# asharakeh/bayes-od-rc

Measured on AMD Instinct MI355X. Metric: images/sec at N=10 MC samples, 512x512; per-anchor covariance latency, higher is better.
Workload: dtype bf16; 1 GPU; ResNet-50 RetinaNet + covar head, N=10 MC-dropout, 512x512, full BayesOD pipeline (forward+posterior+soft-NMS+cluster-fuse); global_batch=512, mc_samples=10, anchors=49104, parallelism=one GPU (no exchange; N > 1: image-sharded, one RCCL gather/step), visible_gpus=1, gpu_max_hw_queues=4

## Files before the change

### bayes-od-rc_amd/_lib.py

```python
import ctypes as C
import os

import numpy as np


_HERE = os.path.dirname(os.path.abspath(__file__))
LIB_PATH = os.path.join(_HERE, "lib", "libbayesod_hip.so")
if os.environ.get("BOD_LIB_OVERRIDE"):
    LIB_PATH = os.path.abspath(os.environ["BOD_LIB_OVERRIDE"])

BOD_OK, BOD_ERR_INVALID_ARG, BOD_ERR_HIP, BOD_ERR_OOM, BOD_ERR_NOT_READY, BOD_ERR_NO_DEVICE = range(6)


class BodConfig(C.Structure):
    _fields_ = [
        ("device", C.c_int32), ("image_h", C.c_int32), ("image_w", C.c_int32), ("batch", C.c_int32),
        ("mc_samples", C.c_int32), ("num_classes", C.c_int32), ("anchors_per_location", C.c_int32),
        ("min_level", C.c_int32), ("max_level", C.c_int32), ("dropout_rate", C.c_float),
        ("use_full_covar", C.c_int32), ("dirichlet_non_informative", C.c_int32),
        ("gaussian_isotropic", C.c_int32), ("isotropic_variance", C.c_float),
        ("ranking_method", C.c_int32), ("nms_max_output_size", C.c_int32),
        ("nms_iou_threshold", C.c_float), ("nms_soft_sigma", C.c_float), ("nms_variant", C.c_int32),
        ("num_categorical_draws", C.c_int32), ("has_covar_head", C.c_int32),
        ("kitti_scale_h", C.c_float), ("kitti_scale_w", C.c_float), ("precision", C.c_int32),
        ("mc_sample_base", C.c_int32),
        ("mc_ensemble_size", C.c_int32),
        ("training", C.c_int32),
        ("backbone_depth", C.c_int32),
        ("pipeline_overlap", C.c_int32),
        ("reserved", C.c_int32 * 2),
    ]


class BodSizes(C.Structure):
    _fields_ = [
        ("num_pixels", C.c_int32), ("num_anchors", C.c_int32), ("level_h", C.c_int32 * 8),
        ("level_w", C.c_int32 * 8), ("num_levels", C.c_int32), ("max_detections", C.c_int32),
        ("device_bytes", C.c_int64),
    ]


_F = C.POINTER(C.c_float)
_I = C.POINTER(C.c_int32)
_H = C.c_void_p

SIGNATURES = {
    "bod_version": (C.c_char_p, []),
    "bod_last_error": (C.c_char_p, [_H]),
    "bod_create": (C.c_int, [C.POINTER(BodConfig), C.POINTER(_H)]),
    "bod_destroy": (C.c_int, [_H]),
    "bod_query_sizes": (C.c_int, [_H, C.POINTER(BodSizes)]),
    "bod_update_config": (C.c_int, [_H, C.POINTER(BodConfig)]),
    "bod_load_weight": (C.c_int, [_H, C.c_char_p, C.c_int32, C.POINTER(C.c_int64), C.c_int32, _F]),
    "bod_finalize_weights": (C.c_int, [_H]),
    "bod_set_anchors": (C.c_int, [_H, _F, C.c_int32]),
    "bod_forward": (C.c_int, [_H, C.c_void_p, C.c_int32, C.c_uint64, C.c_uint32]),
    "bod_get_raw": (C.c_int, [_H, _F, _F, _F]),
    "bod_set_raw": (C.c_int, [_H, _F, _F, _F]),
    "bod_get_pyramid": (C.c_int, [_H, C.c_int32, _F]),
    "bod_posterior": (C.c_int, [_H, C.c_uint64, C.c_uint32]),
    "bod_validation_post": (C.c_int, [_H]),
    "bod_get_num_kept": (C.c_int, [_H, _I]),
    "bod_get_posterior": (C.c_int, [_H, C.c_int32, _F, _F, _F, _F, _F, _I]),
    "bod_set_posterior": (C.c_int, [_H, C.c_int32, C.c_int32, _F, _F, _F, _F]),
    "bod_nms": (C.c_int, [_H]),
    "bod_get_nms": (C.c_int, [_H, C.c_int32, _I, _I]),
    "bod_set_nms": (C.c_int, [_H, C.c_int32, _I, C.c_int32]),
    "bod_get_iou_matrix": (C.c_int, [_H, C.c_int32, _F]),
    "bod_cluster_fuse": (C.c_int, [_H]),
    "bod_set_affinity": (C.c_int, [_H, C.c_int32, _F, C.c_int32, C.c_int32]),
    "bod_get_detections": (C.c_int, [_H, C.c_int32, _I, _F, _F, _F, _F]),
    "bod_get_detections_batch": (C.c_int, [_H, _I, _F, _F, _F, _F]),
    "bod_device_detections": (C.c_int, [_H, C.c_int32, C.POINTER(C.c_void_p)]),
    "bod_device_raw": (C.c_int, [_H, C.POINTER(C.c_void_p), C.c_int32]),
    "bod_infer": (C.c_int, [_H, C.c_void_p, C.c_int32, C.c_uint64, C.c_uint32]),
    "bod_infer_async": (C.c_int, [_H, C.c_void_p, C.c_int32, C.c_uint64, C.c_uint32, _I]),
    "bod_collect": (C.c_int, [_H, C.c_int32, _I, _F, _F, _F, _F]),
    "bod_upload_images": (C.c_int, [_H, _F]),
    "bod_upload_frames_u8": (C.c_int, [_H, C.POINTER(C.c_uint8), C.c_int32, C.c_int32, _F, C.c_int32]),
    "bod_upload_frames_u8_async": (C.c_int, [_H, C.POINTER(C.c_uint8), C.c_int32, C.c_int32, _F, C.c_int32, C.c_int32]),
    "bod_device_images_buffer": (C.c_void_p, [_H, C.c_int32]),
    "bod_device_images": (C.c_void_p, [_H]),
    "bod_synchronize": (C.c_int, [_H]),
    "bod_stage_conv_wgrad": (C.c_int, [C.c_int32, _F, C.c_int32, C.c_int32, C.c_int32, C.c_int32, _F, C.c_int32, C.c_int32,
                                       C.c_int32, C.c_int32, C.c_int32, C.c_int32, _F, _F]),
    "bod_stage_conv": (C.c_int, [C.c_int32, _F, C.c_int32, C.c_int32, C.c_int32, C.c_int32, _F, _F,
                                 C.c_int32, C.c_int32, C.c_int32, C.c_int32, C.c_int32, C.c_int32, _F,
                                 C.c_float, C.c_uint64, C.c_int32, C.c_uint32, C.c_int32, C.c_int32, _F]),
    "bod_loss_forward": (C.c_int, [C.c_int32, C.c_int32, C.c_int32, C.c_int32, _F, _F, _F, _F, _F, _F,
                                   C.POINTER(C.c_uint8), C.POINTER(C.c_uint8), C.c_int32, C.c_int32, C.c_float,
                                   C.POINTER(C.c_double)]),
    "bod_train_step": (C.c_int, [_H, C.c_void_p, C.c_int32, _F, _F, C.POINTER(C.c_uint8), C.POINTER(C.c_uint8), C.c_uint64, C.c_uint32,
                                 C.c_int32, C.c_float, C.c_float, C.c_float, C.c_float, C.c_float, C.c_int32, C.POINTER(C.c_double)]),
    "bod_train_gradients": (C.c_int, [_H, C.POINTER(C.c_void_p), C.POINTER(C.c_int64)]),
    "bod_train_apply": (C.c_int, [_H, C.c_float, C.POINTER(C.c_double)]),
    "bod_train_get": (C.c_int, [_H, C.c_char_p, C.c_int32, C.c_int32, _F, C.c_int64]),
    "bod_train_set": (C.c_int, [_H, C.c_char_p, C.c_int32, C.c_int32, _F, C.c_int64]),
    "bod_train_step_count": (C.c_int, [_H, C.POINTER(C.c_int64), C.c_int64]),
    "bod_loss_backward": (C.c_int, [C.c_int32, C.c_int32, C.c_int32, C.c_int32, _F, _F, _F, _F, _F, _F,
                                    C.POINTER(C.c_uint8), C.POINTER(C.c_uint8), C.c_int32, C.c_int32, C.c_float,
                                    C.c_float, C.c_float, C.POINTER(C.c_double), _F, _F, _F]),
    "bod_bench_head_conv": (C.c_int, [_H, C.c_int32, C.c_int32, C.c_int32, C.POINTER(C.c_double), C.POINTER(C.c_double)]),
    "bod_profile_begin": (C.c_int, [_H]),
    "bod_profile_select": (C.c_int, [_H, C.c_int32]),
    "bod_plan_info": (C.c_int, [_H, C.POINTER(C.c_int32)]),
    "bod_record_width": (C.c_int32, [_H]),
    "bod_gather_detections": (C.c_int, [_H, C.c_int32, C.c_void_p, C.c_int32, C.c_int32, C.c_int32, C.c_void_p, C.POINTER(C.c_void_p)]),
    "bod_profile_end": (C.c_int, [_H, C.POINTER(C.c_double), C.POINTER(C.c_int64),
                                  C.POINTER(C.c_double), C.POINTER(C.c_double), C.POINTER(C.c_int64)]),
}

_lib = None


def load():
    global _lib
    if _lib is not None:
        return _lib
    if not os.path.exists(LIB_PATH):
        raise RuntimeError(
            "libbayesod_hip.so not found at %s -- build it with `python -c 'import __graft_entry__ as g; "
            "g.build()'` (there is no CPU fallback)" % LIB_PATH)
    lib = C.CDLL(LIB_PATH)
    for name, (res, args) in SIGNATURES.items():
        fn = getattr(lib, name)
        fn.restype = res
        fn.argtypes = args
    _lib = lib
    return lib


def fptr(a):
    return None if a is None else a.ctypes.data_as(_F)


def iptr(a):
    return None if a is None else a.ctypes.data_as(_I)


def check(lib, handle, status):
    if status == BOD_OK:
        return
    msg = lib.bod_last_error(handle)
    msg = msg.decode() if msg else "status %d" % status
    if status in (BOD_ERR_INVALID_ARG, BOD_ERR_NOT_READY):
        raise ValueError(msg)
    if status == BOD_ERR_OOM:
        raise MemoryError(msg)
    raise RuntimeError(msg)


def as_f32(a):
    return np.ascontiguousarray(a, dtype=np.float32)
```

### bayes-od-rc_amd/csrc/engine.hip

```cpp
#include "../../include/bayesod.h"
#include "kernels.h"

#include <algorithm>
#include <atomic>
#include <cmath>
#include <condition_variable>
#include <deque>
#include <functional>
#include <mutex>
#include <thread>
#include <tuple>
#include <cstdarg>
#include <cstdio>
#include <cstring>
#include <map>
#include <memory>
#include <string>
#include <vector>
#include <dlfcn.h>

namespace {

constexpr float BN_EPS = 1e-3f;

thread_local std::string g_create_error;

struct HostTensor { std::vector<int64_t> shape; std::vector<float> data; };

struct Plane {
    char* d = nullptr;
    int64_t base = 0;
    int64_t bstride = 0;
    int h = 0, w = 0, C = 0, pitch = 0;
};

struct PackedConv { char* w = nullptr; float* bias = nullptr; int cout = 0, cout_pad = 0, taps = 0, kw = 0, cin = 0; };

struct Op {
    enum Kind { STEM, POOL, CONV, KEEP } kind;
    ConvArgs conv;
    bool is_head3x3 = false;
    double flops = 0;
    std::string name;
    std::string wname[3], bnname[3];
    bool same_geom = false;
    int flavour = 0;
    int head[3] = {-1, -1, -1};
    bool hx_pyramid = false;
};
enum { FLAVOUR_BOTH = 0, FLAVOUR_RAW = 1, FLAVOUR_AGG = 2 };

uint16_t f2bf(float f) {
    uint32_t u; std::memcpy(&u, &f, 4);
    u += 0x7FFFu + ((u >> 16) & 1u);
    return (uint16_t)(u >> 16);
}
float bf2f(uint16_t v) { uint32_t u = (uint32_t)v << 16; float f; std::memcpy(&f, &u, 4); return f; }

uint16_t f2h(float f) {
    uint32_t u; std::memcpy(&u, &f, 4);
    const uint32_t sign = (u >> 16) & 0x8000u;
    u &= 0x7FFFFFFFu;
    if (u >= 0x47800000u) return (uint16_t)(sign | (u > 0x7F800000u ? 0x7E00u : 0x7C00u));
    if (u < 0x38800000u) {
        float a; std::memcpy(&a, &u, 4);
        return (uint16_t)(sign | (uint32_t)std::nearbyint(a * 16777216.0f));
    }
    u += 0xFFFu + ((u >> 13) & 1u);
    return (uint16_t)(sign | ((u - 0x38000000u) >> 13));
}
float h2f(uint16_t h) {
    const uint32_t sign = (uint32_t)(h & 0x8000u) << 16, e = (h >> 10) & 31u, m = h & 0x3FFu;
    float f;
    if (e == 0) { f = (float)m * (1.0f / 16777216.0f); uint32_t u; std::memcpy(&u, &f, 4); u |= sign; std::memcpy(&f, &u, 4); return f; }
    const uint32_t u = sign | ((e == 31 ? 255u : e + 112u) << 23) | (m << 13);
    std::memcpy(&f, &u, 4);
    return f;
}
uint32_t f2e2m3(float x) {
    const uint32_t sign = std::signbit(x) ? 32u : 0u;
    const float a = std::fabs(x);
    uint32_t code;
    if (a < 1.0f) code = (uint32_t)std::nearbyint(a * 8.0f);
    else if (a < 2.0f) code = 8u + (uint32_t)std::nearbyint((a - 1.0f) * 8.0f);
    else if (a < 4.0f) code = 16u + (uint32_t)std::nearbyint((a - 2.0f) * 4.0f);
    else code = 24u + (uint32_t)std::nearbyint((std::min(a, 7.5f) - 4.0f) * 2.0f);
    return sign | std::min(code, 31u);
}
float e2m3_to_f(uint32_t c) {
    const uint32_t e = (c >> 3) & 3u, m = c & 7u;
    const float r = e == 0 ? m / 8.0f : std::ldexp(1.0f + m / 8.0f, (int)e - 1);
    return (c & 32u) ? -r : r;
}
void pack_hx_row(const float* v, int C, uint8_t* dst, bool weights) {
    std::memset(dst, 0, (size_t)C * 4);
    for (int q = 0; q < C / 64; ++q) {
        uint8_t* H = dst + (size_t)q * 256;
        uint8_t* X = H + 128;
        for (int c = 0; c < 64; ++c) { const uint16_t hb = f2h(v[q * 64 + c]); std::memcpy(H + 2 * c, &hb, 2); }
        for (int m = 0; m < 2; ++m)
            for (int b = 0; b < 2; ++b) {
                float hi[16], lo[16], mx = 6.103515625e-05f;
                for (int k = 0; k < 16; ++k) {
                    const float x = v[q * 64 + 32 * m + 8 * (k >> 2) + 4 * b + (k & 3)];
                    hi[k] = h2f(f2h(x)); lo[k] = (x - hi[k]) * 2048.0f;
                    mx = std::max(mx, std::fabs(x));
                }
                const float mxs = mx * 1.0666667f;
                uint32_t ub; std::memcpy(&ub, &mxs, 4);
                const uint32_t eb = (ub >> 23) - 2u;
                const float inv = std::ldexp(1.0f, 127 - (int)eb);
                uint8_t slot[32] = {0};
                for (int k = 0; k < 16; ++k) {
                    const uint32_t h6 = f2e2m3(hi[k] * inv), l6 = f2e2m3(lo[k] * inv);
                    const uint32_t e0 = weights ? l6 : h6, e1 = weights ? h6 : l6;
                    const int bit0 = 12 * k;
                    for (int t = 0; t < 6; ++t) {
                        if ((e0 >> t) & 1u) slot[(bit0 + t) >> 3] |= (uint8_t)(1u << ((bit0 + t) & 7));
                        if ((e1 >> t) & 1u) slot[(bit0 + 6 + t) >> 3] |= (uint8_t)(1u << ((bit0 + 6 + t) & 7));
                    }
                }
                slot[28] = (uint8_t)(weights ? eb - 11u : eb);
                std::memcpy(X + 64 * m + 16 * b, slot, 16);
                std::memcpy(X + 64 * m + 32 + 16 * b, slot + 16, 16);
            }
    }
}
void unpack_hx_row(const uint8_t* src, int C, float* v) {
    for (int q = 0; q < C / 64; ++q) {
        const uint8_t* H = src + (size_t)q * 256;
        const uint8_t* X = H + 128;
        for (int m = 0; m < 2; ++m)
            for (int b = 0; b < 2; ++b) {
                uint8_t slot[32];
                std::memcpy(slot, X + 64 * m + 16 * b, 16);
                std::memcpy(slot + 16, X + 64 * m + 32 + 16 * b, 16);
                const float sc = std::ldexp(1.0f, (int)slot[28] - 127);
                for (int k = 0; k < 16; ++k) {
                    const int c = 32 * m + 8 * (k >> 2) + 4 * b + (k & 3);
                    uint16_t hb; std::memcpy(&hb, H + 2 * c, 2);
                    uint32_t l6 = 0;
                    for (int t = 0; t < 6; ++t) l6 |= (uint32_t)((slot[(12 * k + 6 + t) >> 3] >> ((12 * k + 6 + t) & 7)) & 1u) << t;
                    v[q * 64 + c] = h2f(hb) + e2m3_to_f(l6) * sc * (1.0f / 2048.0f);
                }
            }
    }
}

uint32_t f2e2m1(float x) {
    const uint32_t s = std::signbit(x) ? 8u : 0u;
    float a = std::fabs(x);
    if (!(a == a)) return s;
    if (a >= 6.0f) return s | 7u;
    static const float grid[8] = {0.f, 0.5f, 1.f, 1.5f, 2.f, 3.f, 4.f, 6.f};
    uint32_t best = 0;
    for (uint32_t c = 0; c < 7; ++c) {
        const float mid = 0.5f * (grid[c] + grid[c + 1]);
        if (a > mid || (a == mid && (c & 1u))) best = c + 1;
    }
    return s | best;
}
float e2m1_to_f(uint32_t c) {
    static const float grid[8] = {0.f, 0.5f, 1.f, 1.5f, 2.f, 3.f, 4.f, 6.f};
    return (c & 8u) ? -grid[c & 7u] : grid[c & 7u];
}
void pack_h4_row(const float* v, int C, uint8_t* dst, bool weights) {
    std::memset(dst, 0, (size_t)C * 4);
    for (int q = 0; q < C / 64; ++q) {
        uint8_t* H = dst + (size_t)(3 * (q >> 1) + (q & 1)) * 128;
        for (int c = 0; c < 64; ++c) { const uint16_t hb = f2h(v[q * 64 + c]); std::memcpy(H + 2 * c, &hb, 2); }
    }
    for (int x = 0; x < C / 128; ++x)
        for (int ks = 0; ks < 4; ++ks)
            for (int b = 0; b < 2; ++b) {
                float hi[16], lo[16], mx = 6.103515625e-05f;
                for (int k = 0; k < 16; ++k) {
                    const float xv = v[128 * x + 32 * ks + 8 * (k >> 2) + 4 * b + (k & 3)];
                    hi[k] = h2f(f2h(xv)); lo[k] = (xv - hi[k]) * 2048.0f;
                    mx = std::max(mx, std::fabs(hi[k]));
                }
                const float mxs = mx * 1.3333334f;
                uint32_t ub; std::memcpy(&ub, &mxs, 4);
                const uint32_t eb = (ub >> 23) - 2u;
                const float inv = std::ldexp(1.0f, 127 - (int)eb);
                uint8_t* piece = dst + (size_t)(3 * x + 2) * 128 + (2 * ks + b) * 16;
                for (int k = 0; k < 16; ++k) {
                    const uint32_t h4 = f2e2m1(hi[k] * inv), l4 = f2e2m1(lo[k] * inv);
                    piece[k] = (uint8_t)(weights ? (l4 | (h4 << 4)) : (h4 | (l4 << 4)));
                }
                dst[6 * 128 + 8 * x + 4 * b + ks] = (uint8_t)(weights ? eb - 11u : eb);
            }
}
void unpack_h4_row(const uint8_t* src, int C, float* v) {
    for (int x = 0; x < C / 128; ++x)
        for (int ks = 0; ks < 4; ++ks)
            for (int b = 0; b < 2; ++b) {
                const uint8_t* piece = src + (size_t)(3 * x + 2) * 128 + (2 * ks + b) * 16;
                const float sc = std::ldexp(1.0f, (int)src[6 * 128 + 8 * x + 4 * b + ks] - 127);
                for (int k = 0; k < 16; ++k) {
                    const int c = 128 * x + 32 * ks + 8 * (k >> 2) + 4 * b + (k & 3);
                    const int q = c >> 6;
                    uint16_t hb; std::memcpy(&hb, src + (size_t)(3 * (q >> 1) + (q & 1)) * 128 + 2 * (c & 63), 2);
                    v[c] = h2f(hb) + e2m1_to_f((uint32_t)piece[k] >> 4) * sc * (1.0f / 2048.0f);
                }
            }
}

}

struct bod_context {
    bod_config cfg{};
    std::string err;
    hipStream_t stream = nullptr;
    std::vector<void*> allocs;
    std::map<const void*, size_t> alloc_bytes;
    int64_t device_bytes = 0;
    struct TrainState* train = nullptr;

    int sh = 0, sw = 0, ph = 0, pw = 0;
    int ch[6] = {0}, cw[6] = {0};
    int nlev = 0; int lh[8] = {0}, lw[8] = {0};
    int64_t lvl_off[8] = {0};
    int64_t lvl_p0[8] = {0};
    int64_t Ppad = 0; int P = 0, A = 0;

    std::map<std::string, HostTensor> host_w;
    std::map<std::string, PackedConv> packed;
    float* stem_w = nullptr; float* stem_b = nullptr;
    bool weights_ready = false, anchors_ready = false, forward_done = false, posterior_done = false,
         nms_done = false, cluster_done = false;

    float* d_images = nullptr;
    float* splitk_partial = nullptr; size_t splitk_elems = 0;
    uint8_t* d_frames_u8 = nullptr; size_t frames_u8_cap = 0;
    float* d_images_b[2] = {nullptr, nullptr}; uint8_t* d_u8_b[2] = {nullptr, nullptr}; size_t u8_cap_b[2] = {0, 0};
    hipStream_t copy = nullptr;
    hipEvent_t ev_img_ready[2] = {nullptr, nullptr}, ev_img_free[2] = {nullptr, nullptr};
    bool img_ready_pending[2] = {false, false}, img_free_pending[2] = {false, false};
    int cur_img_buf = -1;
    char* stem_out = nullptr;
    int es = 2;
    bool split = false;
    char* pyr_hx = nullptr;
    int pyr_fmt = 1;
    int plan_mx = 0;
    int mx = 0;
    Plane pyramid;
    char* head_act[3][2] = {{nullptr}};
    char* head_act_t[3][4] = {{nullptr}};
    float* raw[3] = {nullptr};
    float* agg[3] = {nullptr};
    bool agg_plan = false;
    bool plan_fused_out = false, plan_xreuse = false, plan_xreuse0 = false;
    bool raw_valid = false, agg_valid = false;
    bool plan_sparse = false;
    SparseTailArgs sparse{};
    bool agg_sparse = false;
    bool keep_ready = false;
    uint64_t keep_seed = 0; uint32_t keep_first = 0;
    uint64_t last_seed = 0; uint32_t last_first_image = 0;
    std::map<std::string, RowEnt*> tables;
    struct XrTable { RowEnt* rows = nullptr; int2* ext = nullptr; int m = 0; };
    std::map<std::string, XrTable> xr_tables;
    std::vector<Op> ops;
    const float* cur_images = nullptr;

    float* d_anchors = nullptr;
    PostBuffers pb{};
    float* nms_scores = nullptr; int32_t* nms_begin = nullptr;
    int32_t* nms_sel_s[2] = {nullptr, nullptr}; int32_t* nms_nsel_s[2] = {nullptr, nullptr};
    float* out_scores_s[2] = {nullptr, nullptr}; float* out_means_s[2] = {nullptr, nullptr};
    float* out_covs_s[2] = {nullptr, nullptr}; float* out_counts_s[2] = {nullptr, nullptr};
    int32_t* nms_sel = nullptr; int32_t* nms_nsel = nullptr;
    float* out_scores = nullptr; float* out_means = nullptr; float* out_covs = nullptr; float* out_counts = nullptr;
    int slot = 0;
    hipStream_t side = nullptr;
    int overlap_mode = 0;
    int ov_front_slots = 0, ov_slots = 0;
    hipStream_t full = nullptr, front = nullptr, back = nullptr;
    hipEvent_t ev_front_done[2] = {nullptr, nullptr}, ev_l0_done[2] = {nullptr, nullptr}, ev_join = nullptr;
    bool l0_pending[2] = {false, false};
    bool ov_dirty = false;
    char* pyr_d[2] = {nullptr, nullptr};
    int fwd_parity = 0, pyr_last = 0;
    int first_head_op = 0;
    bool in_overlap_call = false;
    int n_cu = 256;
    hipEvent_t ev_posterior = nullptr; hipEvent_t ev_done[2] = {nullptr, nullptr};
    int dev_op_lo = 0, dev_op_hi = 1 << 30;
    hipStream_t done_stream[2] = {nullptr, nullptr};
    bool side_pending[2] = {false, false};
    char* host_stage[2] = {nullptr, nullptr};
    float* rec_send = nullptr; float* rec_recv = nullptr; size_t rec_recv_elems = 0;
    hipEvent_t ev_gather = nullptr; hipStream_t gather_stream = nullptr;
    void select_slot(int sidx) {
        slot = sidx;
        nms_sel = nms_sel_s[sidx]; nms_nsel = nms_nsel_s[sidx];
        out_scores = out_scores_s[sidx]; out_means = out_means_s[sidx];
        out_covs = out_covs_s[sidx]; out_counts = out_counts_s[sidx];
    }
    float* iou_scratch = nullptr; int64_t iou_cap = 0;
    float* affinity = nullptr; int affinity_img = -1;

    bool profiling = false; int prof_which = 0;
    std::vector<std::pair<hipEvent_t, hipEvent_t>> ev_head, ev_post;
    double prof_flops = 0;

    bod_status fail(bod_status s, const char* fmt, ...) {
        char buf[1024];
        va_list ap; va_start(ap, fmt); vsnprintf(buf, sizeof buf, fmt, ap); va_end(ap);
        err = buf;
        return s;
    }
    template <typename T> bod_status dalloc(T** p, size_t n_elems, bool zero = true) {
        void* q = nullptr;
        const size_t bytes = std::max<size_t>(n_elems * sizeof(T), 256);
        hipError_t e = hipMalloc(&q, bytes);
        if (e != hipSuccess) return fail(BOD_ERR_OOM, "hipMalloc(%zu) failed: %s", bytes, hipGetErrorString(e));
        if (zero) {
            e = hipMemsetAsync(q, 0, bytes, stream);
            if (e != hipSuccess) return fail(BOD_ERR_HIP, "hipMemset: %s", hipGetErrorString(e));
        }
        allocs.push_back(q);
        alloc_bytes[q] = bytes;
        device_bytes += (int64_t)bytes;
        *p = reinterpret_cast<T*>(q);
        return BOD_OK;
    }
};

#define HIPCHK(h, expr)                                                                         \
    do {                                                                                        \
        hipError_t _e = (expr);                                                                 \
        if (_e != hipSuccess)                                                                   \
            return (h)->fail(BOD_ERR_HIP, "%s failed: %s (%s:%d)", #expr, hipGetErrorString(_e), \
                             __FILE__, __LINE__);                                               \
    } while (0)
#define BODCHK(expr) do { bod_status _s = (expr); if (_s != BOD_OK) return _s; } while (0)

namespace {

const char* kHeadPrefix[3] = {"pyramid_classification", "pyramid_regression", "pyramid_cov"};
const int kHeadConvs[3] = {4, 3, 4};

void cu_slot_mask(int lo, int hi, uint32_t mask[8]) {
    for (int w = 0; w < 8; ++w) mask[w] = 0u;
    for (int slot = lo; slot < hi; ++slot)
        for (int xcd = 0; xcd < 8; ++xcd) { const int bit = slot * 8 + xcd; mask[bit >> 5] |= 1u << (bit & 31); }
}

int same_pad_before(int in, int k, int s) {
    const int out = (in + s - 1) / s;
    const int total = std::max((out - 1) * s + k - in, 0);
    return total / 2;
}

bod_status new_plane(bod_context* h, Plane* p, int B, int hh, int ww, int C) {
    p->h = hh; p->w = ww; p->C = C; p->pitch = ww + 2; p->base = 0;
    p->bstride = (int64_t)(hh + 2) * (ww + 2);
    return h->dalloc(&p->d, (size_t)B * p->bstride * C * h->es);
}

bod_status make_table(bod_context* h, const std::string& key, int B, const Plane& in, const Plane& out,
                      int stride, int org_y, int org_x, const Plane* res, const RowEnt** tbl) {
    auto it = h->tables.find(key);
    if (it != h->tables.end()) { *tbl = it->second; return BOD_OK; }
    std::vector<RowEnt> rows((size_t)B * out.h * out.w);
    size_t r = 0;
    for (int b = 0; b < B; ++b)
        for (int y = 0; y < out.h; ++y)
            for (int x = 0; x < out.w; ++x) {
                RowEnt e{};
                e.in_off = (int32_t)(in.base + b * in.bstride + (int64_t)(y * stride + org_y) * in.pitch + (x * stride + org_x));
                e.in_pitch = in.pitch;
                e.out_off = (int32_t)(out.base + b * out.bstride + (int64_t)(y + 1) * out.pitch + (x + 1));
                if (res) {
                    int ry = y, rx = x;
                    if (res->h != out.h || res->w != out.w) {
                        ry = std::min((int)std::floor((y + 0.5) * ((double)res->h / out.h)), res->h - 1);
                        rx = std::min((int)std::floor((x + 0.5) * ((double)res->w / out.w)), res->w - 1);
                    }
                    e.res_off = (int32_t)(res->base + b * res->bstride + (int64_t)(ry + 1) * res->pitch + (rx + 1));
                }
                rows[r++] = e;
            }
    RowEnt* d = nullptr;
    BODCHK(h->dalloc(&d, rows.size(), false));
    HIPCHK(h, hipMemcpyAsync(d, rows.data(), rows.size() * sizeof(RowEnt), hipMemcpyHostToDevice, h->stream));
    HIPCHK(h, hipStreamSynchronize(h->stream));
    h->tables[key] = d;
    *tbl = d;
    return BOD_OK;
}

const HostTensor* find_w(bod_context* h, const std::string& name, int kind) {
    auto it = h->host_w.find(name + "/" + std::to_string(kind));
    return it == h->host_w.end() ? nullptr : &it->second;
}

bod_status pack_conv(bod_context* h, const std::string& name, const std::string& bn, int cout_pad_to,
                     PackedConv* out, int hx = 0) {
    const std::string ckey = hx == 2 ? name + ":h4" : hx ? name + ":hx" : name;
    auto it = h->packed.find(ckey);
    if (it != h->packed.end()) { *out = it->second; return BOD_OK; }
    const HostTensor* k = find_w(h, name, 0);
    if (!k || k->shape.size() != 4) return h->fail(BOD_ERR_NOT_READY, "missing conv kernel '%s'", name.c_str());
    const int kh = (int)k->shape[0], kw = (int)k->shape[1], cin = (int)k->shape[2], cout = (int)k->shape[3];
    const HostTensor* b = find_w(h, name, 1);
// ... 306 lines not shown
                    Plane fresh;
                    BODCHK(new_plane(h, &fresh, B, hh, ww, f3));
                    x = out;
                    if (use_a) oa = fresh; else ob = fresh;
                    use_a = !use_a;
                    continue;
                }
                x = out;
                use_a = !use_a;
                continue;
            }
            auto fuse_next_2a = [&](const char* blk) -> bod_status {
                if (st != 2 || blk[1] == 0 || train_mode || h->es != 2 || h->split) return BOD_OK;
                Op& op2c = h->ops.back();
                if (!conv_pointwise_can_fuse_next(op2c.conv) || op2c.conv.ksplit > 1) return BOD_OK;
                char nb[64], nbb[64];
                snprintf(nb, sizeof nb, "res%d%c_branch2a", st, blk[1]);
                snprintf(nbb, sizeof nbb, "bn%d%c_branch2a", st, blk[1]);
                PackedConv p2a;
                BODCHK(pack_conv(h, nb, nbb, 64, &p2a));
                if (p2a.cin != f3 || p2a.cout != f1 || p2a.taps != 1 || p2a.cout_pad != 64) return BOD_OK;
                ConvGroup& G = op2c.conv.g[0];
                G.ch_w3 = p2a.w; G.ch_b3 = p2a.bias; G.ch_out3 = t1.d;
                op2c.flops += 2.0 * op2c.conv.M * (double)f1 * f3;
                op2c.name += std::string("+") + nb; op2c.wname[2] = nb; op2c.bnname[2] = nbb;
                pw_t1_ready = true;
                return BOD_OK;
            };
            if (train_mode) {
                BODCHK(new_plane(h, &t1, B, hh, ww, f1));
                BODCHK(new_plane(h, &t2, B, hh, ww, f1));
                BODCHK(new_plane(h, &sc, B, hh, ww, f3));
                BODCHK(new_plane(h, &oa, B, hh, ww, f3));
                BODCHK(new_plane(h, &ob, B, hh, ww, f3));
            }
            Plane& out = use_a ? oa : ob;
            if (*bl == 'a') {
                bool dual = false;
                if (st == 2 && !train_mode && h->es == 2 && !h->split) {
                    BODCHK(add_conv(h, c_ + "1", b_ + "1", x, sc, first_stride, false, false, nullptr));
                    Op& op1 = h->ops.back();
                    PackedConv p2a;
                    BODCHK(pack_conv(h, c_ + "2a", b_ + "2a", 64, &p2a));
                    if (conv_pointwise_can_fuse_dual(op1.conv) && op1.conv.ksplit <= 1 && p2a.cin == 64 && p2a.cout == f1 && f1 == 64 &&
                        p2a.taps == 1 && p2a.cout_pad == 64) {
                        ConvGroup& G = op1.conv.g[0];
                        G.ch_w3 = p2a.w; G.ch_b3 = p2a.bias; G.ch_out3 = t1.d; G.ch_dual = 1;
                        op1.flops += 2.0 * op1.conv.M * (double)f1 * 64.0;
                        op1.name += std::string("+") + c_ + "2a"; op1.wname[2] = c_ + "2a"; op1.bnname[2] = b_ + "2a";
                        dual = true;
                    } else {
                        h->ops.pop_back();
                    }
                }
                if (!dual) BODCHK(add_conv(h, c_ + "2a", b_ + "2a", x, t1, first_stride, false, true, nullptr));
                BODCHK(add_conv(h, c_ + "2b", b_ + "2b", t1, t2, 1, true, true, nullptr));
                if (!dual) BODCHK(add_conv(h, c_ + "1", b_ + "1", x, sc, first_stride, false, false, nullptr));
                BODCHK(add_conv(h, c_ + "2c", b_ + "2c", t2, out, 1, false, true, &sc));
                BODCHK(fuse_next_2a(bl));
                if (st == 3 || st == 4) {
                    taps[st] = out;
                    Plane fresh;
                    BODCHK(new_plane(h, &fresh, B, hh, ww, f3));
                    x = out;
                    if (use_a) oa = fresh; else ob = fresh;
                    use_a = !use_a;
                    continue;
                }
            } else {
                if (!pw_t1_ready) BODCHK(add_conv(h, c_ + "2a", b_ + "2a", x, t1, 1, false, true, nullptr));
                pw_t1_ready = false;
                BODCHK(add_conv(h, c_ + "2b", b_ + "2b", t1, t2, 1, true, true, nullptr));
                BODCHK(add_conv(h, c_ + "2c", b_ + "2c", t2, out, 1, false, true, &x));
                BODCHK(fuse_next_2a(bl));
            }
            x = out;
            use_a = !use_a;
        }
    }
    const Plane c5 = x, c4 = taps[4], c3 = taps[3];

    h->pyramid.C = 256; h->pyramid.bstride = h->Ppad;
    BODCHK(h->dalloc(&h->pyramid.d, (size_t)B * h->Ppad * 256 * h->es));
    Plane c5r, m4, m3, p6relu;
    BODCHK(new_plane(h, &c5r, B, h->lh[2], h->lw[2], 256));
    BODCHK(new_plane(h, &m4, B, h->lh[1], h->lw[1], 256));
    BODCHK(new_plane(h, &m3, B, h->lh[0], h->lw[0], 256));
    char* p6relu_buf = nullptr;
    BODCHK(h->dalloc(&p6relu_buf, (size_t)B * h->Ppad * 256 * h->es));
    p6relu = h->pyramid; p6relu.d = p6relu_buf;
    BODCHK(add_conv(h, "C5_reduced", "", c5, c5r, 1, false, false, nullptr));
    BODCHK(add_conv(h, "P5", "", c5r, level_view(h, 2), 1, true, false, nullptr));
    BODCHK(add_conv(h, "P6", "", c5, level_view(h, 3), 2, true, false, nullptr, p6relu_buf));
    {
        Plane v = p6relu; v.base = h->lvl_off[3]; v.h = h->lh[3]; v.w = h->lw[3]; v.pitch = h->lw[3] + 2;
        BODCHK(add_conv(h, "P7", "", v, level_view(h, 4), 2, true, false, nullptr));
    }
    BODCHK(add_conv(h, "C4_reduced", "", c4, m4, 1, false, false, &c5r));
    BODCHK(add_conv(h, "P4", "", m4, level_view(h, 1), 1, true, false, nullptr));
    BODCHK(add_conv(h, "C3_reduced", "", c3, m3, 1, false, false, &m4));
    BODCHK(add_conv(h, "P3", "", m3, level_view(h, 0), 1, true, false, nullptr));

    const size_t act_elems = (size_t)B * N * h->Ppad * 256 * h->es;
    for (int hd = 0; hd < 3; ++hd) {
        if (hd == 2 && !c.has_covar_head) continue;
        if (train_mode) {
            for (int l = 0; l < kHeadConvs[hd]; ++l) BODCHK(h->dalloc(&h->head_act_t[hd][l], act_elems));
            continue;
        }
        BODCHK(h->dalloc(&h->head_act[hd][0], act_elems));
        BODCHK(h->dalloc(&h->head_act[hd][1], act_elems));
    }
    const int out_ch[3] = {c.anchors_per_location * c.num_classes, c.anchors_per_location * 4, c.anchors_per_location * 10};
    std::vector<RowEnt> t1, t2, t3;
    {
        PyramidGeometry pg = pyramid_geometry(h->lh, h->lw);
        if (pg.Ppad != h->Ppad || pg.P != h->P) return h->fail(BOD_ERR_INVALID_ARG, "pyramid geometry mismatch");
        head_row_tables(pg, B, N, t1, t2, t3);
    }
    RowEnt *d1 = nullptr, *d2 = nullptr, *d3 = nullptr;
    BODCHK(h->dalloc(&d1, t1.size(), false));
    BODCHK(h->dalloc(&d2, t2.size(), false));
    BODCHK(h->dalloc(&d3, t3.size(), false));
    HIPCHK(h, hipMemcpyAsync(d1, t1.data(), t1.size() * sizeof(RowEnt), hipMemcpyHostToDevice, h->stream));
    HIPCHK(h, hipMemcpyAsync(d2, t2.data(), t2.size() * sizeof(RowEnt), hipMemcpyHostToDevice, h->stream));
    HIPCHK(h, hipMemcpyAsync(d3, t3.data(), t3.size() * sizeof(RowEnt), hipMemcpyHostToDevice, h->stream));
    HIPCHK(h, hipStreamSynchronize(h->stream));

    RowEnt* d2x = nullptr; int2* dext = nullptr; int m2x = 0;
    bool xreuse = (h->es == 2 || h->split) && !train_mode;
    if (const char* e = getenv("BOD_CONV_XREUSE")) xreuse = xreuse && atoi(e) != 0;
    bool mx_plan = h->mx != 0 && xreuse;
    const int mxf = h->mx;
    if (const char* e = getenv("BOD_TOWER_MX")) mx_plan = mx_plan && atoi(e) != 0;
    {
        ConvArgs probe{};
        probe.M = B * N * h->P; probe.cout_pad = 256; probe.fan_count = 1; probe.flags = CONV_RELU;
        xreuse = xreuse && (mx_plan || conv_igemm_uses_full_cout_tile(probe));
    }
    static_assert(sizeof(ExtRow) == sizeof(int2), "ExtRow is the host-side twin of int2");
    auto make_xr_tiles = [&](const std::vector<RowEnt>& src, RowEnt** d_rows, int2** d_ext, int* m_out) -> bod_status {
        std::vector<RowEnt> tiled;
        std::vector<ExtRow> ext;
        if (!xr_tile_rows(src, tiled, ext)) return h->fail(BOD_ERR_INVALID_ARG, "row-reuse tiling: extended rows out of order");
        *m_out = (int)tiled.size();
        BODCHK(h->dalloc(d_rows, tiled.size(), false));
        BODCHK(h->dalloc(d_ext, ext.size(), false));
        HIPCHK(h, hipMemcpyAsync(*d_rows, tiled.data(), tiled.size() * sizeof(RowEnt), hipMemcpyHostToDevice, h->stream));
        HIPCHK(h, hipMemcpyAsync(*d_ext, ext.data(), ext.size() * sizeof(int2), hipMemcpyHostToDevice, h->stream));
        HIPCHK(h, hipStreamSynchronize(h->stream));
        return BOD_OK;
    };
    if (xreuse) BODCHK(make_xr_tiles(t2, &d2x, &dext, &m2x));
    RowEnt* d1x = nullptr; int2* dext1 = nullptr; int m1x = 0;
    bool xreuse0 = xreuse;
    if (const char* e = getenv("BOD_FAN_XREUSE")) xreuse0 = xreuse0 && atoi(e) != 0;
    {
        ConvArgs probe{};
        probe.M = B * h->P; probe.cout_pad = 256; probe.fan_count = N; probe.flags = CONV_RELU | CONV_DROPOUT; probe.groups = c.has_covar_head ? 3 : 2;
        xreuse0 = xreuse0 && conv_igemm_uses_full_cout_tile(probe);
    }
    if (mx_plan) xreuse0 = true;
    bool mx_l0 = mx_plan && !c.pipeline_overlap;
    if (const char* e = getenv("BOD_MX_LAYER0")) mx_l0 = mx_l0 && atoi(e) != 0;
    if (mx_l0) BODCHK(h->dalloc(&h->pyr_hx, (size_t)B * h->Ppad * 256 * 4));
    if (xreuse0) BODCHK(make_xr_tiles(t1, &d1x, &dext1, &m1x));

    const bool mc = train_mode || std::max(N, c.mc_ensemble_size) > 1;
    const uint32_t thr = (uint32_t)std::floor((double)c.dropout_rate * 65536.0);
    const float dscale = (float)(1.0 / (1.0 - (double)c.dropout_rate));
    const int nheads = c.has_covar_head ? 3 : 2;
    bool fuse_out = (h->es == 2 || (h->split && xreuse)) && !train_mode;
    if (const char* e = getenv("BOD_FUSE_HEAD_OUTPUT")) fuse_out = fuse_out && atoi(e) != 0;
    {
        ConvArgs probe{};
        probe.M = B * N * h->P; probe.cout_pad = 256; probe.fan_count = 1; probe.flags = CONV_RELU;
        fuse_out = fuse_out && (mx_plan || conv_igemm_uses_full_cout_tile(probe));
    }
    bool agg = xreuse && fuse_out && N >= 2 && 256 / N >= 1 && 320 / N - 2 >= 1 && c.mc_ensemble_size <= N;
    if (const char* e = getenv("BOD_FUSE_AGGREGATION")) agg = agg && atoi(e) != 0;
    RowEnt* d2a = nullptr; int2* dexta = nullptr; int m2a = 0;
    if (agg) {
        std::vector<RowEnt> tiled;
        std::vector<ExtRow> ext;
        const int rc = xr_tile_rows_aggregated(t2, B, N, h->P, tiled, ext);
        if (rc == 1) return h->fail(BOD_ERR_INVALID_ARG, "aggregated tiling: no pixel fits a tile (N = %d)", N);
        if (rc == 2) return h->fail(BOD_ERR_INVALID_ARG, "aggregated tiling: extended rows out of order");
        m2a = (int)tiled.size();
        BODCHK(h->dalloc(&d2a, tiled.size(), false));
        BODCHK(h->dalloc(&dexta, ext.size(), false));
        HIPCHK(h, hipMemcpyAsync(d2a, tiled.data(), tiled.size() * sizeof(RowEnt), hipMemcpyHostToDevice, h->stream));
        HIPCHK(h, hipMemcpyAsync(dexta, ext.data(), ext.size() * sizeof(int2), hipMemcpyHostToDevice, h->stream));
        HIPCHK(h, hipStreamSynchronize(h->stream));
        const size_t BA = (size_t)B * h->A;
        BODCHK(h->dalloc(&h->agg[0], BA * c.num_classes));
        BODCHK(h->dalloc(&h->agg[1], BA * 16));
        if (c.has_covar_head) BODCHK(h->dalloc(&h->agg[2], BA * 10));
    } else {
        BODCHK(ensure_raw(h));
    }
    static const bool split_on = [] { const char* e = getenv("BOD_SPLIT_AGG_LAUNCH"); return !e || atoi(e) != 0; }();
    bool sparse = agg && split_on && h->es == 2 && !h->split && !mx_plan && !c.pipeline_overlap && h->A == h->P * c.anchors_per_location &&
                  h->P <= 65536;
    if (const char* e = getenv("BOD_SPARSE_TAIL")) sparse = sparse && atoi(e) != 0;
    if (sparse) {
        SparseTailArgs& sa = h->sparse;
        sa.B = B; sa.N = N; sa.P = h->P; sa.apl = c.anchors_per_location; sa.Ppad = h->Ppad;
        sa.cap_tiles = B * (h->P / sparse_tail_min_pixels(N) + 1);
        RowEnt* pix = nullptr;
        BODCHK(h->dalloc(&pix, (size_t)h->P, false));
        HIPCHK(h, hipMemcpyAsync(pix, t2.data(), (size_t)h->P * sizeof(RowEnt), hipMemcpyHostToDevice, h->stream));
        HIPCHK(h, hipStreamSynchronize(h->stream));
        sa.pix = pix;
        BODCHK(h->dalloc(&sa.rows, (size_t)sa.cap_tiles * 256, false));
        BODCHK(h->dalloc(&sa.ext, (size_t)sa.cap_tiles * XR_EXT_ROWS, false));
        BODCHK(h->dalloc(&sa.tile_count, 1));
        BODCHK(h->dalloc(&sa.chunks, (size_t)B * h->P, false));
        BODCHK(h->dalloc(&sa.tiles, (size_t)B * h->P, false));
    }
    h->plan_sparse = sparse;
    Op sparse_op; sparse_op.kind = Op::CONV; sparse_op.is_head3x3 = true; sparse_op.flavour = FLAVOUR_AGG;
    int sparse_groups = 0; PackedConv sparse_pc{};
    h->agg_plan = agg; h->plan_fused_out = fuse_out; h->plan_xreuse = xreuse; h->plan_xreuse0 = xreuse0; h->plan_mx = mx_plan ? mxf : 0;
    int hfmt[3] = {mxf, mxf, mxf};
    if (mxf == 2) { const char* e = getenv("BOD_MX4_BOX_HX"); if (e && atoi(e) != 0) hfmt[1] = 1; }
    if (mxf == 1) { static const bool cls_h4 = [] { const char* e = getenv("BOD_MX_CLS_H4"); return !e || atoi(e) != 0; }(); if (cls_h4) hfmt[0] = 2; }
    const bool mixed = mx_plan && hfmt[0] != hfmt[1];
    const int pyr_fmt = mixed ? 1 : mxf;
    h->pyr_fmt = pyr_fmt;
    for (int layer = 0; layer < 4; ++layer)
    for (int fpass = 0; fpass < 2; ++fpass)
    for (int part = 0; part < 2; ++part)
    for (int flav = (agg && layer >= 2) ? FLAVOUR_RAW : FLAVOUR_BOTH; flav <= ((agg && layer >= 2) ? FLAVOUR_AGG : FLAVOUR_BOTH); ++flav) {
        const bool split_launch = agg && layer >= 2 && split_on;
        if (fpass == 1 && (!mixed || layer == 0)) continue;
        const int lfmt = !mx_plan ? 0 : layer == 0 ? pyr_fmt : mixed ? (fpass == 0 ? 2 : 1) : mxf;
        if (!split_launch && part == 1) continue;
        if (split_launch && part == 0 && flav == FLAVOUR_AGG) continue;
        const bool both = split_launch && part == 0;
        Op op; op.kind = Op::CONV; op.is_head3x3 = true; op.flavour = both ? FLAVOUR_BOTH : flav;
        int g = 0; PackedConv pc0{};
        double fused_flops = 0;
        for (int hd = 0; hd < nheads; ++hd) {
            if (layer >= kHeadConvs[hd]) continue;
            if (split_launch && (part == 1) != (layer == kHeadConvs[hd] - 1)) continue;
            if (mixed && layer > 0 && hfmt[hd] != lfmt) continue;
            PackedConv pc;
            BODCHK(pack_conv(h, std::string(kHeadPrefix[hd]) + "_" + std::to_string(layer), "", 128, &pc, (mx_plan && (layer > 0 || mx_l0)) ? lfmt : 0));
            if (pc.cin != 256 || pc.cout != 256 || pc.taps != 9)
                return h->fail(BOD_ERR_INVALID_ARG, "head conv %s_%d must be 3x3 256->256", kHeadPrefix[hd], layer);
            op.wname[g] = std::string(kHeadPrefix[hd]) + "_" + std::to_string(layer);
            ConvGroup cg{};
            cg.in = layer == 0 ? (mx_l0 ? h->pyr_hx : h->pyramid.d) : (train_mode ? h->head_act_t[hd][layer - 1] : h->head_act[hd][(layer + 1) & 1]);
            cg.w = pc.w; cg.bias = pc.bias;
            cg.out = train_mode ? h->head_act_t[hd][layer] : h->head_act[hd][layer & 1];
            cg.layer_id = hd * 4 + layer;
            cg.out_hx = (mx_plan && layer < kHeadConvs[hd] - 1) ? hfmt[hd] : 0;
            if (fuse_out && layer == kHeadConvs[hd] - 1) {
                PackedConv po;
                BODCHK(pack_conv(h, kHeadPrefix[hd], "", 32, &po));
                if (po.cin != 256 || po.cout != out_ch[hd] || po.taps != 1)
                    return h->fail(BOD_ERR_INVALID_ARG, "head output conv %s must be 1x1 256->%d (got %d->%d)", kHeadPrefix[hd], out_ch[hd], po.cin, po.cout);
                cg.w2 = po.w; cg.bias2 = po.bias; cg.out2 = h->raw[hd]; cg.cout2 = po.cout; cg.out2_cstride = out_ch[hd];
                op.head[g] = hd;
                if (flav == FLAVOUR_AGG) {
                    cg.out2 = nullptr;
                    cg.agg_kind = hd == 0 ? AGG_CLS : hd == 1 ? AGG_BOX : AGG_COV;
                    cg.agg_n = N; cg.agg_P = h->P; cg.agg_C = c.num_classes; cg.agg_out = h->agg[hd]; cg.anchors = h->d_anchors;
                }
                fused_flops += 2.0 * ((double)B * N * h->P) * 256.0 * out_ch[hd];
            }
            if (sparse && flav == FLAVOUR_AGG && hd != 0) {
                sparse_op.conv.g[sparse_groups] = cg;
                sparse_op.wname[sparse_groups] = op.wname[g];
                sparse_op.head[sparse_groups] = hd;
                if (sparse_groups++ == 0) sparse_pc = pc;
                sparse_op.flops += 2.0 * ((double)B * N * h->P) * 256.0 * 2304.0 + 2.0 * ((double)B * N * h->P) * 256.0 * out_ch[hd];
                fused_flops -= 2.0 * ((double)B * N * h->P) * 256.0 * out_ch[hd];
                op.head[g] = -1; op.wname[g].clear();
                continue;
            }
            op.conv.g[g] = cg;
            if (g == 0) pc0 = pc;
            ++g;
        }
        if (g == 0) continue;
        const int M = layer == 0 ? B * h->P : B * N * h->P;
        ConvArgs a = base_args(pc0, layer == 0 ? d1 : d2, M, 256, 256);
        for (int q = 0; q < g; ++q) a.g[q] = op.conv.g[q];
        a.groups = g;
        a.flags = CONV_RELU | (mc ? CONV_DROPOUT : 0);
        a.fan_count = layer == 0 ? N : 1;
        a.fan_stride = (int32_t)h->Ppad;
        a.drop_threshold = thr; a.drop_scale = dscale;
        a.mx = mx_plan ? ((layer == 0 && !mx_l0) ? 2 : (lfmt == 2 ? 3 : 1)) : 0;
        op.hx_pyramid = mx_l0 && layer == 0;
        {
            static const int mx_loader = getenv("BOD_MX_LOADER") ? atoi(getenv("BOD_MX_LOADER")) : 1;
            static const int tower_loader = getenv("BOD_TOWER_LOADER") ? atoi(getenv("BOD_TOWER_LOADER")) : 0;
            a.mx_loader = mx_plan ? mx_loader : ((h->es == 2 && layer > 0) ? tower_loader : 0);
        }
        if (xreuse0 && layer == 0) { a.rows = d1x; a.M = m1x; a.ext = dext1; a.xreuse = 2; }
        if (xreuse && layer > 0) {
            a.rows = d2x; a.M = m2x; a.ext = dext;
            if (agg && layer >= 2 && !(split_launch && part == 0)) { a.rows = d2a; a.M = m2a; a.ext = dexta; }
            a.xreuse = 2;
        }
        op.conv = a;
        op.flops = 2.0 * M * 256.0 * 2304.0 * g + fused_flops;
        op.name = "head_tower_layer_" + std::to_string(layer) + (both ? "" : flav == FLAVOUR_AGG ? "(aggregating)" : flav == FLAVOUR_RAW ? "(raw)" : "");
        op.same_geom = N == 1;
        h->ops.push_back(op);
    }
    if (sparse_groups > 0) {
        Op keep; keep.kind = Op::KEEP; keep.flavour = FLAVOUR_AGG; keep.name = "head_tower_layer_3(keep)";
        h->ops.push_back(keep);
        const SparseTailArgs& sa = h->sparse;
        ConvArgs a = base_args(sparse_pc, sa.rows, sa.cap_tiles * 256, 256, 256);
        for (int q = 0; q < sparse_groups; ++q) a.g[q] = sparse_op.conv.g[q];
        a.groups = sparse_groups;
        a.flags = CONV_RELU | (mc ? CONV_DROPOUT : 0);
        a.fan_count = 1; a.fan_stride = (int32_t)h->Ppad;
        a.drop_threshold = thr; a.drop_scale = dscale;
        a.ext = sa.ext; a.xreuse = 2; a.tile_count = sa.tile_count;
        a.mx_loader = getenv("BOD_TOWER_LOADER") ? atoi(getenv("BOD_TOWER_LOADER")) : 0;
        sparse_op.conv = a;
        sparse_op.name = "head_tower_layer_3(sparse)";
        h->ops.push_back(sparse_op);
    }
    for (int hd = 0; hd < nheads && !fuse_out; ++hd) {
        PackedConv pc;
        BODCHK(pack_conv(h, kHeadPrefix[hd], "", 64, &pc));
        if (pc.cin != 256 || pc.cout != out_ch[hd] || pc.taps != 1)
            return h->fail(BOD_ERR_INVALID_ARG, "head output conv %s must be 1x1 256->%d (got %d->%d)", kHeadPrefix[hd], out_ch[hd], pc.cin, pc.cout);
        Op op; op.kind = Op::CONV;
        ConvArgs a = base_args(pc, d3, B * N * h->P, 256, out_ch[hd]);
        a.g[0] = ConvGroup{train_mode ? h->head_act_t[hd][kHeadConvs[hd] - 1] : h->head_act[hd][(kHeadConvs[hd] - 1) & 1], pc.w, pc.bias, h->raw[hd], nullptr, nullptr, 0, 0, nullptr, nullptr, nullptr, 0, 0};
        a.flags = CONV_OUT_F32;
        op.conv = a;
        op.flops = 2.0 * a.M * pc.cout * 256.0;
        op.name = kHeadPrefix[hd]; op.wname[0] = kHeadPrefix[hd];
        h->ops.push_back(op);
    }
    if (h->splitk_elems) {
        BODCHK(h->dalloc(&h->splitk_partial, h->splitk_elems));
        for (Op& o : h->ops) if (o.kind == Op::CONV && o.conv.ksplit > 1) o.conv.partial = h->splitk_partial;
    }
    if (h->split) for (Op& o : h->ops) if (o.kind == Op::CONV) to_split_args(&o.conv);
    h->first_head_op = (int)h->ops.size();
    for (size_t i = 0; i < h->ops.size(); ++i) if (h->ops[i].is_head3x3) { h->first_head_op = (int)i; break; }
    h->pyr_d[0] = h->pyramid.d;
    if (const char* e = getenv("BOD_DUMP_OPS")) if (atoi(e) != 0) {
        fprintf(stderr, "# ops: index name kind flavour M taps cin cout groups fan has_res fused_next flops bytes\n");
        for (size_t i = 0; i < h->ops.size(); ++i) {
            const Op& o = h->ops[i];
            const ConvArgs& a = o.conv;
            double bytes = 0;
            if (o.kind == Op::STEM)
                bytes = (double)B * c.image_h * c.image_w * 3 * 4 + (double)B * h->ph * h->pw * 64 * h->es;
            if (o.kind == Op::CONV) {
                const double es = (a.flags & CONV_OUT_F32) ? 4.0 : (double)h->es;
                for (int g = 0; g < a.groups; ++g) {
                    bytes += (double)a.M * a.cin * h->es;
                    bytes += (double)a.M * std::max(1, a.fan_count) * a.cout_valid * es;
                    if (a.g[g].res) bytes += (double)a.M * a.cout_valid * h->es;
                    if (a.g[g].ch_w3) bytes += (double)a.M * 64 * h->es;
                    bytes += (double)a.taps * a.cin * a.cout_pad * h->es;
                }
            }
            fprintf(stderr, "# op %zu %s %d %d %d %d %d %d %d %d %d %d %.6g %.6g\n", i, o.name.c_str(), (int)o.kind, o.flavour, a.M, a.taps, a.cin,
                    a.cout_valid, a.groups, a.fan_count, o.kind == Op::CONV && a.g[0].res ? 1 : 0, o.kind == Op::CONV && a.g[0].ch_w3 ? 1 : 0, o.flops, bytes);
        }
    }
    if (h->overlap_mode) BODCHK(h->dalloc(&h->pyr_d[1], (size_t)B * h->Ppad * 256 * h->es));
    return BOD_OK;
}

bod_status alloc_post(bod_context* h) {
    const bod_config& c = h->cfg;
    const size_t BA = (size_t)c.batch * h->A;
    const int nblocks = (h->A + 255) / 256;
    PostBuffers& p = h->pb;
    BODCHK(h->dalloc(&p.keep, BA));
    BODCHK(h->dalloc(&p.d_counts, BA * c.num_classes));
    BODCHK(h->dalloc(&p.block_counts, (size_t)c.batch * nblocks));
    BODCHK(h->dalloc(&p.num_kept, (size_t)c.batch));
    BODCHK(h->dalloc(&p.counts, BA * c.num_classes));
    BODCHK(h->dalloc(&p.score, BA * c.num_classes));
    BODCHK(h->dalloc(&p.means, BA * 4));
    BODCHK(h->dalloc(&p.covs, BA * 16));
    BODCHK(h->dalloc(&p.ranking, BA));
    BODCHK(h->dalloc(&p.corners, BA * 4));
    BODCHK(h->dalloc(&p.anchor_index, BA));
    BODCHK(h->dalloc(&h->d_anchors, (size_t)h->A * 4));
    const size_t BApad = (size_t)h->cfg.batch * ((h->A + 511) & ~(size_t)511);
    BODCHK(h->dalloc(&h->nms_scores, BApad));
    BODCHK(h->dalloc(&h->nms_begin, BApad));
    const size_t BK = (size_t)c.batch * c.nms_max_output_size;
    for (int sidx = 0; sidx < 2; ++sidx) {
        BODCHK(h->dalloc(&h->nms_sel_s[sidx], BK));
        BODCHK(h->dalloc(&h->nms_nsel_s[sidx], (size_t)c.batch));
        BODCHK(h->dalloc(&h->out_scores_s[sidx], BK * c.num_classes));
        BODCHK(h->dalloc(&h->out_means_s[sidx], BK * 4));
        BODCHK(h->dalloc(&h->out_covs_s[sidx], BK * 16));
        BODCHK(h->dalloc(&h->out_counts_s[sidx], BK * c.num_classes));
        const size_t stage_bytes = ((size_t)c.batch + BK * (2 * (size_t)c.num_classes + 20)) * 4;
        if (hipHostMalloc(reinterpret_cast<void**>(&h->host_stage[sidx]), stage_bytes, hipHostMallocDefault) != hipSuccess)
            return h->fail(BOD_ERR_OOM, "pinned host staging buffer (%zu bytes)", stage_bytes);
    }
    h->select_slot(0);
    BODCHK(h->dalloc(&h->d_images, (size_t)c.batch * c.image_h * c.image_w * 3));
    h->d_images_b[0] = h->d_images;
    return BOD_OK;
}

PostCfg post_cfg(bod_context* h, uint64_t seed, uint32_t first_image) {
    const bod_config& c = h->cfg;
    PostCfg p{};
    p.B = c.batch; p.N = c.mc_samples; p.A = h->A; p.C = c.num_classes; p.draws = c.num_categorical_draws;
    p.use_full_covar = c.use_full_covar; p.has_covar = c.has_covar_head; p.dirichlet = c.dirichlet_non_informative;
    p.gaussian_iso = c.gaussian_isotropic; p.ranking_method = c.ranking_method; p.iso_var = c.isotropic_variance;
    p.kitti_sh = c.kitti_scale_h; p.kitti_sw = c.kitti_scale_w;
    p.seed_lo = (uint32_t)seed; p.seed_hi = (uint32_t)(seed >> 32); p.image_base = first_image;
    return p;
}

struct Markers {
    bool on = false;
    int (*push)(const char*) = nullptr;
    int (*pop)() = nullptr;
    Markers() {
        const char* e = getenv("BOD_ROCTX");
        if (!e || !atoi(e)) return;
        void* lib = dlopen("librocprofiler-sdk-roctx.so", RTLD_NOW | RTLD_GLOBAL);
        if (!lib) lib = dlopen("libroctx64.so", RTLD_NOW | RTLD_GLOBAL);
        if (!lib) { fprintf(stderr, "bayesod: BOD_ROCTX=1 but no roctx library could be opened (%s)\n", dlerror()); return; }
        push = reinterpret_cast<int (*)(const char*)>(dlsym(lib, "roctxRangePushA"));
        pop = reinterpret_cast<int (*)()>(dlsym(lib, "roctxRangePop"));
        on = push && pop;
    }
};
static Markers& markers() { static Markers m; return m; }
struct MarkerRange {
    bool on;
    explicit MarkerRange(const char* name) : on(markers().on) { if (on) markers().push(name); }
    ~MarkerRange() { if (on) markers().pop(); }
    MarkerRange(const MarkerRange&) = delete;
    MarkerRange& operator=(const MarkerRange&) = delete;
};
static std::string op_stage(const std::string& name) {
    if (name.rfind("conv1", 0) == 0 || name.rfind("pool1", 0) == 0) return "bod:stem";
    if (name.rfind("res", 0) == 0 && name.size() > 3) return "bod:" + name.substr(0, 4);
    if (name.rfind("head_tower_layer_", 0) == 0) return "bod:" + name.substr(0, name.find('(') == std::string::npos ? name.size() : name.find('('));
    if (name.rfind("pyramid_", 0) == 0) return "bod:head_outputs";
    return "bod:fpn";
}

bod_status mark_images_consumed(bod_context* h, hipStream_t st = nullptr) {
    if (h->cur_img_buf >= 0 && h->copy) {
        HIPCHK(h, hipEventRecord(h->ev_img_free[h->cur_img_buf], st ? st : h->stream));
        h->img_free_pending[h->cur_img_buf] = true;
    }
    return BOD_OK;
}

bod_status join_overlap(bod_context* h) {
    if (!h->ov_dirty) return BOD_OK;
    HIPCHK(h, hipStreamSynchronize(h->front));
    HIPCHK(h, hipStreamSynchronize(h->back));
    h->ov_dirty = false;
    return BOD_OK;
}

bod_status run_forward(bod_context* h, const float* dev_images, uint64_t seed, uint32_t first_image, int flavour = FLAVOUR_RAW,
                       bool only_flavoured = false, bool overlapped = false) {
    const bod_config& c = h->cfg;
    if (flavour == FLAVOUR_RAW && !only_flavoured) BODCHK(ensure_raw(h));
    const bool ov = overlapped && h->overlap_mode != 0 && !only_flavoured;
    hipStream_t fs = ov ? h->front : h->stream;
    int par = 0;
    if (ov) {
        par = h->fwd_parity; h->fwd_parity ^= 1;
        if (h->l0_pending[par]) { HIPCHK(h, hipStreamWaitEvent(fs, h->ev_l0_done[par], 0)); h->l0_pending[par] = false; }
    }
    if (!only_flavoured) { h->pyr_last = par; h->keep_ready = false; }
    const int cus_front = h->n_cu;
    const int cus_back = h->n_cu;
    static const int trace_call = getenv("BOD_TRACE_OPS") ? atoi(getenv("BOD_TRACE_OPS")) : 0;
    static int call_no = 0;
    const bool trace = trace_call > 0 && ++call_no == trace_call && !ov;
    std::vector<hipEvent_t> tev;
    if (trace) {
        tev.resize(h->ops.size() + 1);
        for (hipEvent_t& e : tev) HIPCHK(h, hipEventCreate(&e));
        HIPCHK(h, hipEventRecord(tev[0], h->stream));
    }
    size_t op_i = 0;
    bool stem_pool_fused = false;
    std::string cur_stage;
    struct StageCloser { std::string& s; ~StageCloser() { if (!s.empty()) markers().pop(); } } stage_closer{cur_stage};
    for (Op& op : h->ops) {
        if (trace && op_i > 0) HIPCHK(h, hipEventRecord(tev[op_i], h->stream));
        const bool is_front = (int)op_i < h->first_head_op;
        const bool first_back = (int)op_i == h->first_head_op;
        hipStream_t st = is_front ? fs : h->stream;
        ++op_i;
        if ((op.flavour != FLAVOUR_BOTH && op.flavour != flavour) || (only_flavoured && op.flavour == FLAVOUR_BOTH)) continue;
        if ((int)op_i - 1 < h->dev_op_lo || (int)op_i - 1 >= h->dev_op_hi) continue;
        if (ov && first_back) {
            HIPCHK(h, hipEventRecord(h->ev_front_done[par], fs));
            HIPCHK(h, hipStreamWaitEvent(h->stream, h->ev_front_done[par], 0));
        }
        if (markers().on) {
            std::string st = op_stage(op.name);
            if (st != cur_stage) {
                if (!cur_stage.empty()) markers().pop();
                markers().push(st.c_str());
                cur_stage.swap(st);
            }
        }
        switch (op.kind) {
            case Op::STEM: {
                const Op* pool = op_i < h->ops.size() && h->ops[op_i].kind == Op::POOL ? &h->ops[op_i] : nullptr;
                static const bool split_fused = [] { const char* e = getenv("BOD_STEM_SPLIT_FUSED"); return !e || atoi(e) != 0; }();
                stem_pool_fused = pool && !h->train && (h->split ? split_fused : h->es == 2) && !trace &&
                                  stem_pool_fused_applies(dev_images, c.batch, c.image_w, h->sw, is_front ? cus_front : cus_back);
                if (stem_pool_fused)
                    HIPCHK(h, launch_stem_pool_fused(dev_images, h->stem_w, h->stem_b, pool->conv.g[0].out, h->split ? 1 : 0, c.batch, c.image_h,
                                                     c.image_w, h->sh, h->sw, h->ph, h->pw, h->pw + 2, (h->ph + 2) * (h->pw + 2), st));
                else
                HIPCHK(h, launch_stem_conv(dev_images, h->stem_w, h->stem_b, h->stem_out, h->es == 4, c.batch, c.image_h,
                                           c.image_w, h->sh, h->sw, st));
                if (!h->train) BODCHK(mark_images_consumed(h, st));
                break;
            }
            case Op::KEEP: {
                for (int sidx = 0; sidx < 2; ++sidx)
                    if (h->side_pending[sidx]) HIPCHK(h, hipStreamWaitEvent(st, h->ev_done[sidx], 0));
                PostCfg pc = post_cfg(h, seed, first_image);
                pc.aggregated = 1;
                PostBuffers pb = h->pb;
                pb.agg_cls = h->agg[0];
                HIPCHK(h, launch_posterior_keep(pc, pb, st));
                SparseTailArgs sa = h->sparse;
                sa.keep = h->pb.keep;
                HIPCHK(h, launch_sparse_tail_rows(sa, st));
                h->keep_ready = true; h->keep_seed = seed; h->keep_first = first_image;
                break;
            }
            case Op::POOL:
                if (stem_pool_fused) break;
                HIPCHK(h, launch_stem_pool(h->stem_out, op.conv.g[0].out, h->split ? 2 : (h->es == 4 ? 1 : 0), c.batch,
                                           h->sh, h->sw, h->ph, h->pw, h->pw + 2, (h->ph + 2) * (h->pw + 2), st));
                break;
            case Op::CONV: {
                if (op.hx_pyramid) HIPCHK(h, launch_pairs_to_hx(h->pyramid.d, h->pyr_hx, (long)c.batch * h->Ppad, 256, st, h->pyr_fmt));
                op.conv.seed_lo = (uint32_t)seed; op.conv.seed_hi = (uint32_t)(seed >> 32);
                op.conv.image_base = first_image;
                op.conv.sample_base = (uint32_t)c.mc_sample_base;
                op.conv.dyn_rng = train_dyn_rng(h);
                const bool is_tower = op.conv.xreuse != 0 && op.conv.fan_count <= 1;
                const bool timed = h->profiling && op.is_head3x3 && (h->prof_which == 0 || (h->prof_which == 1) == is_tower);
                hipEvent_t e0 = nullptr, e1 = nullptr;
                if (timed) {
                    HIPCHK(h, hipEventCreate(&e0)); HIPCHK(h, hipEventCreate(&e1));
                    HIPCHK(h, hipEventRecord(e0, st));
                }
                op.conv.n_cu = is_front ? cus_front : cus_back;
                {
                    static const int stagger_us = getenv("BOD_FAN_STAGGER_US") ? atoi(getenv("BOD_FAN_STAGGER_US")) : 0;
                    op.conv.stagger_ticks = (op.conv.fan_count > 1 && op.conv.xreuse) ? stagger_us * 100 : 0;
                }
                if (par != 0) {
                    ConvArgs a = op.conv;
                    for (int g = 0; g < a.groups; ++g) {
                        if (a.g[g].in == h->pyr_d[0]) a.g[g].in = h->pyr_d[1];
                        if (a.g[g].out == h->pyr_d[0]) a.g[g].out = h->pyr_d[1];
                    }
                    HIPCHK(h, (h->es == 4 && !h->split) ? launch_conv_igemm_f32(a, st) : launch_conv_igemm(a, st));
                } else
                HIPCHK(h, (h->es == 4 && !h->split) ? launch_conv_igemm_f32(op.conv, st) : launch_conv_igemm(op.conv, st));
                if (timed) {
                    HIPCHK(h, hipEventRecord(e1, st));
                    h->ev_head.emplace_back(e0, e1);
                    h->prof_flops += op.flops;
                }
                if (ov && first_back) {
                    HIPCHK(h, hipEventRecord(h->ev_l0_done[par], h->stream));
                    h->l0_pending[par] = true;
                }
                break;
            }
        }
    }
    if (trace) {
        HIPCHK(h, hipEventRecord(tev[h->ops.size()], h->stream));
        HIPCHK(h, hipStreamSynchronize(h->stream));
        fprintf(stderr, "# op trace: name kind M taps cin cout_pad groups fan ms TFLOP/s\n");
        for (size_t i = 0; i < h->ops.size(); ++i) {
            float ms = 0.f;
            HIPCHK(h, hipEventElapsedTime(&ms, tev[i], tev[i + 1]));
            const Op& o = h->ops[i];
            fprintf(stderr, "%-28s %d %8d %2d %5d %5d %d %2d %9.4f %8.1f\n", o.name.c_str(), (int)o.kind, o.conv.M, o.conv.taps,
                    o.conv.cin, o.conv.cout_pad, o.conv.groups, o.conv.fan_count, ms, o.flops / (ms * 1e-3) / 1e12);
        }
        for (hipEvent_t& e : tev) hipEventDestroy(e);
    }
    h->forward_done = true; h->posterior_done = h->nms_done = h->cluster_done = false; h->affinity_img = -1;
    h->last_seed = seed; h->last_first_image = first_image;
    if (flavour == FLAVOUR_AGG) { h->agg_valid = true; h->raw_valid = false; h->agg_sparse = h->plan_sparse; }
    else { h->raw_valid = true; if (!only_flavoured) h->agg_valid = false; }
    return BOD_OK;
}

bod_status materialise_raw(bod_context* h) {
    if (h->raw_valid || !h->agg_valid) { BODCHK(ensure_raw(h)); return BOD_OK; }
    BODCHK(ensure_raw(h));
    const bool prof = h->profiling;
    h->profiling = false;
    const bool fd = h->forward_done, pd = h->posterior_done, nd = h->nms_done, cd = h->cluster_done;
    const int aff = h->affinity_img;
    const bod_status st = run_forward(h, h->cur_images, h->last_seed, h->last_first_image, FLAVOUR_RAW, true);
    h->profiling = prof;
    h->forward_done = fd; h->posterior_done = pd; h->nms_done = nd; h->cluster_done = cd; h->affinity_img = aff;
    return st;
}

bod_status run_posterior(bod_context* h, uint64_t seed, uint32_t first_image) {
    if (!h->anchors_ready) return h->fail(BOD_ERR_NOT_READY, "bod_set_anchors has not been called");
    for (int sidx = 0; sidx < 2; ++sidx)
        if (h->side_pending[sidx]) HIPCHK(h, hipStreamWaitEvent(h->stream, h->ev_done[sidx], 0));
    MarkerRange mr("bod:posterior");
    PostCfg pc = post_cfg(h, seed, first_image);
    PostBuffers pb = h->pb;
    pb.cls = h->raw[0]; pb.box = h->raw[1]; pb.cov = h->raw[2]; pb.anchors = h->d_anchors;
    pc.aggregated = (h->agg_valid && !h->raw_valid) ? 1 : 0;
    pb.agg_cls = h->agg[0]; pb.agg_box = h->agg[1]; pb.agg_cov = h->agg[2];
    const bool keep_done = pc.aggregated && h->keep_ready && seed == h->keep_seed && first_image == h->keep_first;
    h->keep_ready = false;
    if (pc.aggregated && h->agg_sparse && (seed != h->keep_seed || first_image != h->keep_first)) {
        BODCHK(materialise_raw(h));
        pc.aggregated = 0;
        pb.cls = h->raw[0]; pb.box = h->raw[1]; pb.cov = h->raw[2];
    }
    hipEvent_t e0 = nullptr, e1 = nullptr;
    if (h->profiling) {
        HIPCHK(h, hipEventCreate(&e0)); HIPCHK(h, hipEventCreate(&e1));
        HIPCHK(h, hipEventRecord(e0, h->stream));
    }
    HIPCHK(h, keep_done ? launch_posterior_fuse(pc, pb, h->stream) : launch_posterior(pc, pb, h->stream));
    if (h->cfg.ranking_method == BOD_RANK_JOINT_ENTROPY && h->cfg.gaussian_isotropic && h->cfg.dirichlet_non_informative)
        HIPCHK(h, launch_joint_entropy_rank(pc, pb, h->stream));
    if (h->profiling) { HIPCHK(h, hipEventRecord(e1, h->stream)); h->ev_post.emplace_back(e0, e1); }
    h->posterior_done = true; h->nms_done = h->cluster_done = false; h->affinity_img = -1;
    return BOD_OK;
}

bod_status run_nms(bod_context* h, hipStream_t st) {
    MarkerRange mr("bod:nms");
    const bod_config& c = h->cfg;
    NmsArgs a{};
    a.B = c.batch; a.A = h->A; a.num_kept = h->pb.num_kept; a.corners = h->pb.corners; a.ranking = h->pb.ranking;
    a.work_scores = h->nms_scores; a.work_begin = h->nms_begin; a.selected = h->nms_sel; a.num_selected = h->nms_nsel;
    a.max_out = c.nms_max_output_size; a.iou_thr = c.nms_iou_threshold; a.sigma = c.nms_soft_sigma; a.variant = c.nms_variant;
    HIPCHK(h, launch_nms(a, st));
    h->nms_done = true; h->cluster_done = false; h->affinity_img = -1;
    return BOD_OK;
}

bod_status run_cluster(bod_context* h, hipStream_t st) {
    MarkerRange mr("bod:cluster_fuse");
    const bod_config& c = h->cfg;
    ClusterArgs a{};
    a.B = c.batch; a.A = h->A; a.C = c.num_classes; a.max_out = c.nms_max_output_size;
    a.num_kept = h->pb.num_kept; a.selected = h->nms_sel; a.num_selected = h->nms_nsel;
    a.corners = h->pb.corners; a.counts = h->pb.counts; a.means = h->pb.means; a.covs = h->pb.covs;
    a.thr = c.nms_iou_threshold;
    a.affinity = h->affinity_img >= 0 ? h->affinity : nullptr; a.affinity_img = h->affinity_img;
    h->affinity_img = -1;
    a.out_scores = h->out_scores; a.out_means = h->out_means; a.out_covs = h->out_covs; a.out_counts = h->out_counts;
    HIPCHK(h, launch_cluster_fuse(a, st));
    h->cluster_done = true;
    return BOD_OK;
}

bod_status stage_images(bod_context* h, const float* images, int on_device, const float** dev, hipStream_t st = nullptr) {
    if (!images) return h->fail(BOD_ERR_INVALID_ARG, "images is NULL");
    if (!st) st = h->stream;
    h->cur_img_buf = -1;
    if (on_device) {
        for (int k = 0; k < 2; ++k)
            if (images == h->d_images_b[k] && h->d_images_b[k]) {
                h->cur_img_buf = k;
                if (h->img_ready_pending[k]) {
                    HIPCHK(h, hipStreamWaitEvent(st, h->ev_img_ready[k], 0));
                    h->img_ready_pending[k] = false;
                }
            }
        *dev = images;
        return BOD_OK;
// ... 1098 lines not shown
    if (!op) return h->fail(BOD_ERR_INVALID_ARG, "no head launch %d", layer);
    ConvArgs a = op->conv;
    a.variant = variant;
    if (const char* z = getenv("BOD_BENCH_ZERO")) {
        if (atoi(z) != 0 && layer > 0) {
            const size_t bytes = (size_t)h->cfg.batch * h->cfg.mc_samples * h->Ppad * 256 * h->es;
            for (int g = 0; g < a.groups; ++g) HIPCHK(h, hipMemsetAsync(const_cast<void*>(a.g[g].in), 0, bytes, h->stream));
        }
    }
    hipEvent_t e0, e1;
    HIPCHK(h, hipEventCreate(&e0)); HIPCHK(h, hipEventCreate(&e1));
    HIPCHK(h, launch_conv_igemm(a, h->stream));
    HIPCHK(h, hipEventRecord(e0, h->stream));
    for (int i = 0; i < iters; ++i) HIPCHK(h, launch_conv_igemm(a, h->stream));
    HIPCHK(h, hipEventRecord(e1, h->stream));
    HIPCHK(h, hipStreamSynchronize(h->stream));
    float ms = 0; HIPCHK(h, hipEventElapsedTime(&ms, e0, e1));
    hipEventDestroy(e0); hipEventDestroy(e1);
    if ((variant == 90 || variant == 91) && a.mx == 1) {
        unsigned long long c[16];
        conv_igemm_phase_cycles(c, true);
        const double tiles = (double)c[15];
        fprintf(stderr, "# f16mx phase clock, wave 0, cycles per tile (%.0f tiles): whole tile %.0f = set-up %.0f + loop %.0f (of which: waiting for the next K-tile's pieces + barrier %.0f, "
                        "K-tile bodies %.0f; 72 K-tiles) + epilogue %.0f; of the wait: vmcnt / lgkmcnt %.0f, s_barrier %.0f\n", tiles, (double)c[9] / tiles, ((double)c[8] - (double)c[6] - (double)c[7]) / tiles,
                ((double)c[6] + (double)c[7]) / tiles, (double)c[6] / tiles, (double)c[7] / tiles, ((double)c[9] - (double)c[8]) / tiles,
                (double)c[13] / tiles, ((double)c[6] - (double)c[13]) / tiles);
        fprintf(stderr, "# f16mx phase clock by K-tile flavour, cycles per K-tile: wave 0: H %.0f  X %.0f | wave 4: H %.0f  X %.0f, wait + barrier per K-tile %.0f (wave 0: %.0f)"
                        " | MFMA issue of a SIMD's two waves: H 2048, X 1024\n",
                (double)c[0] / tiles / 36.0, (double)c[1] / tiles / 36.0, (double)c[2] / tiles / 36.0, (double)c[3] / tiles / 36.0, (double)c[4] / tiles / 72.0, (double)c[6] / tiles / 72.0);
    } else if (variant == 90) {
        unsigned long long c[16];
        conv_igemm_phase_cycles(c, true);
        const double tiles = (double)c[15];
        static const char* names[6] = {"set-up", "main loop", "barrier+bias/relu/pack", "philox+lds writes", "barrier", "store loop"};
        fprintf(stderr, "# phase clock, wave 0, cycles per tile (%.0f tiles):", tiles);
        for (int k = 0; k < 6; ++k) fprintf(stderr, "  %s %.0f", names[k], (double)c[k] / tiles);
        if (c[10] + c[11] + c[12] > 0)
            fprintf(stderr, "  fused 1x1 MFMAs %.0f  barriers+fp32 tile %.0f  MC reduction+stores %.0f", (double)c[10] / tiles, (double)c[11] / tiles, (double)c[12] / tiles);
        double cyc = 0; for (int k = 0; k < 6; ++k) cyc += (double)c[k];
        cyc += (double)c[10] + (double)c[11] + (double)c[12];
        fprintf(stderr, "  | shader clock during the tiles %.3f GHz (cycles / 100 MHz real-time ticks); tiles account for %.3f ms of the %.3f ms launch per CU\n",
                cyc / (double)c[14] * 0.1, (double)c[14] / tiles * 1e-5 * (tiles / (iters + 1)) / 256.0, ms / iters);
    }
    *mean_ms = ms / iters;
    if (flops) *flops = op->flops;
    return BOD_OK;
}

bod_status bod_profile_begin(bod_handle h) {
    if (!h) return BOD_ERR_INVALID_ARG;
    for (auto& e : h->ev_head) { hipEventDestroy(e.first); hipEventDestroy(e.second); }
    for (auto& e : h->ev_post) { hipEventDestroy(e.first); hipEventDestroy(e.second); }
    h->ev_head.clear(); h->ev_post.clear(); h->prof_flops = 0; h->profiling = true;
    return BOD_OK;
}

extern "C++" {
namespace {
struct Rccl {
    typedef int (*gather_fn)(const void*, void*, size_t, int, int, void*, hipStream_t);
    typedef const char* (*errstr_fn)(int);
    gather_fn gather = nullptr; errstr_fn errstr = nullptr; bool tried = false;
    bool load() {
        if (tried) return gather != nullptr;
        tried = true;
        void* lib = dlopen("librccl.so", RTLD_NOW | RTLD_GLOBAL);
        if (!lib) lib = dlopen("librccl.so.1", RTLD_NOW | RTLD_GLOBAL);
        if (!lib) return false;
        gather = reinterpret_cast<gather_fn>(dlsym(lib, "ncclGather"));
        errstr = reinterpret_cast<errstr_fn>(dlsym(lib, "ncclGetErrorString"));
        return gather != nullptr;
    }
};
Rccl& rccl() { static Rccl r; return r; }
}
}

int32_t bod_record_width(bod_handle h) { return h ? 21 + 2 * h->cfg.num_classes : 0; }

bod_status bod_gather_detections(bod_handle h, int32_t slot, void* nccl_comm, int32_t world, int32_t rank, int32_t root,
                                 float* gathered_host, float** gathered_device) {
    MarkerRange mr_api("bod:gather_detections");
    if (!h) return BOD_ERR_INVALID_ARG;
    if (world < 1 || rank < 0 || rank >= world || root < 0 || root >= world)
        return h->fail(BOD_ERR_INVALID_ARG, "bod_gather_detections: world %d, rank %d, root %d", world, rank, root);
    if (!nccl_comm && world != 1) return h->fail(BOD_ERR_INVALID_ARG, "bod_gather_detections: %d ranks need an ncclComm_t", world);
    if (rank != root && (gathered_host || gathered_device)) return h->fail(BOD_ERR_INVALID_ARG, "bod_gather_detections: only the root receives");
    HIPCHK(h, hipSetDevice(h->cfg.device));
    const int B = h->cfg.batch, K = h->cfg.nms_max_output_size, C = h->cfg.num_classes, W = 21 + 2 * C;
    const size_t block = (size_t)B * K * W;
    int sidx = slot;
    static const bool side_on = [] { const char* e = getenv("BOD_SIDE_STREAM"); return e && atoi(e) != 0; }();
    hipStream_t st = (slot >= 0 && slot <= 1 && !side_on && h->done_stream[slot]) ? h->done_stream[slot] : h->side;
    if (slot < 0) {
        if (!h->cluster_done) return h->fail(BOD_ERR_NOT_READY, "bod_gather_detections: bod_cluster_fuse has not run");
        BODCHK(join_overlap(h));
        sidx = h->slot;
        st = h->stream;
    } else if (slot > 1 || !h->side_pending[slot]) {
        return h->fail(BOD_ERR_NOT_READY, "bod_gather_detections: slot %d has no pending batch", slot);
    }
    if (!h->rec_send && hipMalloc(reinterpret_cast<void**>(&h->rec_send), block * 4) != hipSuccess)
        return h->fail(BOD_ERR_OOM, "bod_gather_detections: %zu bytes", block * 4);
    if (h->ev_gather && h->gather_stream && h->gather_stream != st) HIPCHK(h, hipStreamWaitEvent(st, h->ev_gather, 0));
    if (slot >= 0) HIPCHK(h, hipStreamWaitEvent(st, h->ev_done[slot], 0));
    HIPCHK(h, launch_pack_records(h->nms_nsel_s[sidx], h->out_scores_s[sidx], h->out_means_s[sidx], h->out_covs_s[sidx],
                                  h->out_counts_s[sidx], h->rec_send, B, K, C, st));
    float* recv = nullptr;
    if (rank == root) {
        if (world == 1 && !nccl_comm) recv = h->rec_send;
        else {
            if (h->rec_recv_elems < block * world) {
                if (h->rec_recv && h->rec_recv != h->rec_send) hipFree(h->rec_recv);
                h->rec_recv = nullptr; h->rec_recv_elems = 0;
                if (hipMalloc(reinterpret_cast<void**>(&h->rec_recv), block * world * 4) != hipSuccess)
                    return h->fail(BOD_ERR_OOM, "bod_gather_detections: %zu bytes", block * world * 4);
                h->rec_recv_elems = block * world;
            }
            recv = h->rec_recv;
        }
    }
    if (nccl_comm) {
        if (!rccl().load()) return h->fail(BOD_ERR_NOT_READY, "bod_gather_detections: librccl.so (ncclGather) could not be opened");
        const int rc = rccl().gather(h->rec_send, recv, block,  7, root, nccl_comm, st);
        if (rc != 0) return h->fail(BOD_ERR_HIP, "ncclGather: %s", rccl().errstr ? rccl().errstr(rc) : "error");
    }
    if (!h->ev_gather) HIPCHK(h, hipEventCreateWithFlags(&h->ev_gather, hipEventDisableTiming));
    if (rank == root && gathered_host) {
        HIPCHK(h, hipMemcpyAsync(gathered_host, recv, block * world * 4, hipMemcpyDeviceToHost, st));
        HIPCHK(h, hipEventRecord(h->ev_gather, st)); h->gather_stream = st;
        HIPCHK(h, hipEventSynchronize(h->ev_gather));
    } else {
        HIPCHK(h, hipEventRecord(h->ev_gather, st)); h->gather_stream = st;
    }
    if (!(rank == root && gathered_host) && slot >= 0) {
        HIPCHK(h, hipEventRecord(h->ev_done[slot], st));
    }
    if (gathered_device) *gathered_device = recv;
    return BOD_OK;
}

bod_status bod_plan_info(bod_handle h, int32_t* info8) {
    if (!h || !info8) return BOD_ERR_INVALID_ARG;
    if (!h->weights_ready) return h->fail(BOD_ERR_NOT_READY, "bod_plan_info: the plan is built by bod_finalize_weights");
    for (int i = 0; i < 8; ++i) info8[i] = 0;
    info8[0] = h->agg_plan; info8[1] = h->plan_fused_out; info8[2] = h->plan_xreuse; info8[3] = h->plan_xreuse0;
    info8[4] = (int32_t)h->ops.size();
    for (const Op& o : h->ops) if (o.kind == Op::CONV && !o.is_head3x3 && o.conv.xreuse) ++info8[5];
    info8[6] = h->plan_mx;
    info8[7] = h->plan_sparse;
    return BOD_OK;
}

bod_status bod_profile_select(bod_handle h, int32_t which) {
    if (!h) return BOD_ERR_INVALID_ARG;
    if (which < 0 || which > 2) return h->fail(BOD_ERR_INVALID_ARG, "bod_profile_select: %d", which);
    h->prof_which = which;
    return BOD_OK;
}

bod_status bod_profile_end(bod_handle h, double* head_ms, int64_t* head_launches, double* head_flops, double* post_ms, int64_t* post_launches) {
    if (!h) return BOD_ERR_INVALID_ARG;
    BODCHK(join_overlap(h));
    HIPCHK(h, hipStreamSynchronize(h->stream));
    double hm = 0, pm = 0;
    for (auto& e : h->ev_head) { float ms = 0; HIPCHK(h, hipEventElapsedTime(&ms, e.first, e.second)); hm += ms; }
    for (auto& e : h->ev_post) { float ms = 0; HIPCHK(h, hipEventElapsedTime(&ms, e.first, e.second)); pm += ms; }
    if (head_ms) *head_ms = hm;
    if (head_launches) *head_launches = (int64_t)h->ev_head.size();
    if (head_flops) *head_flops = h->prof_flops;
    if (post_ms) *post_ms = pm;
    if (post_launches) *post_launches = (int64_t)h->ev_post.size();
    h->profiling = false;
    return BOD_OK;
}

}

#include "train_impl.inc"
```

### bayes-od-rc_amd/csrc/kernels.h

```cpp
#pragma once
#include <hip/hip_runtime.h>
#include <stdint.h>
#include "plan_tables.h"


struct ConvGroup {
    const void* in;
    const void* w;
    const float* bias;
    void* out;
    const void* res;
    void* out_relu;
    int32_t in_coff;
    int32_t layer_id;
    const void* w2;
    const float* bias2;
    float* out2;
    int32_t cout2;
    int32_t out2_cstride;
    int32_t agg_kind;
    int32_t agg_n;
    int32_t agg_P;
    int32_t agg_C;
    float* agg_out;
    const float* anchors;
    const void* ch_w2; const float* ch_b2; const void* ch_res; void* ch_out; int32_t ch_c2;
    const void* ch_w3; const float* ch_b3; void* ch_out3;
    int32_t ch_dual;
    int32_t out_hx;
};
enum : int32_t { AGG_NONE = 0, AGG_CLS = 1, AGG_BOX = 2, AGG_COV = 3 };

enum : int32_t { CONV_RELU = 1, CONV_DROPOUT = 2, CONV_OUT_F32 = 4,
                 CONV_ACCUM = 8,
                 CONV_NT_OUT = 16 };

struct ConvArgs {
    ConvGroup g[3];
    const RowEnt* rows;
    int32_t M;
    int32_t taps, KW;
    int32_t cin;
    int32_t in_cstride;
    int32_t cout_pad;
    int32_t cout_valid;
    int32_t out_cstride;
    int32_t res_cstride;
    int32_t flags;
    int32_t fan_count;
    int32_t fan_stride;
    uint32_t seed_lo, seed_hi;
    uint32_t drop_threshold;
    float drop_scale;
    uint32_t image_base;
    int32_t groups;
    int32_t variant;
    const int2* ext;
    int32_t xreuse;
    int32_t ksplit;
    float* partial;
    const uint32_t* dyn_rng;
    uint32_t sample_base;
    int32_t split;
    int32_t plane_h, plane_w;
    int32_t n_cu;
    int32_t stagger_ticks;
    int32_t fan_chunk;
    int32_t mx;
    int32_t mx_loader;
    const int32_t* tile_count;
};

struct PerDeviceOnce {
    bool done[64] = {false};
    bool* slot() { int d = 0; if (hipGetDevice(&d) != hipSuccess || d < 0 || d >= 64) d = 0; return &done[d]; }
};

int device_cu_count();
inline int launch_cus(const ConvArgs& a) { return a.n_cu > 0 ? a.n_cu : device_cu_count(); }
hipError_t launch_conv_igemm(const ConvArgs& a, hipStream_t s);
bool conv_igemm_uses_full_cout_tile(const ConvArgs& a);
bool conv_igemm_uses_big_tile(const ConvArgs& a);
void conv_igemm_phase_cycles(unsigned long long* out16, bool reset);
hipError_t launch_conv_igemm_f32(const ConvArgs& a, hipStream_t s);
hipError_t launch_pairs_to_hx(const void* in, void* out, long npix, int C, hipStream_t s, int fmt = 1);

hipError_t launch_stem_conv(const float* img, const float* w, const float* bias, void* out, int out_f32,
                            int B, int H, int W, int oh, int ow, hipStream_t s);
bool stem_pool_fused_applies(const float* img, int B, int W, int ow, int n_cu);
hipError_t launch_stem_pool_fused(const float* img, const float* w, const float* bias, void* pooled, int split, int B, int H, int W, int oh,
                                  int ow, int ph, int pw, int pool_pitch, int pool_plane, hipStream_t s);
hipError_t launch_stem_pool(const void* in, void* out, int mode, int B, int ih, int iw, int oh, int ow,
                            int out_pitch, int out_plane, hipStream_t s);

struct PostCfg {
    int32_t B, N, A, C, draws;
    int32_t use_full_covar, has_covar, dirichlet, gaussian_iso, ranking_method;
    float iso_var;
    float kitti_sh, kitti_sw;
    uint32_t seed_lo, seed_hi, image_base;
    int32_t aggregated;
};

struct PostBuffers {
    const float* cls;
    const float* box;
    const float* cov;
    const float* anchors;
    const float* agg_cls;
    const float* agg_box;
    const float* agg_cov;
    uint8_t* keep;
    float* d_counts;
    int32_t* block_counts;
    int32_t* num_kept;
    float* counts;
    float* score;
    float* means;
    float* covs;
    float* ranking;
    float* corners;
    int32_t* anchor_index;
};

hipError_t launch_posterior(const PostCfg& c, const PostBuffers& b, hipStream_t s);
hipError_t launch_posterior_keep(const PostCfg& c, const PostBuffers& b, hipStream_t s);
hipError_t launch_posterior_fuse(const PostCfg& c, const PostBuffers& b, hipStream_t s);

struct SparseTailArgs {
    const uint8_t* keep;
    const RowEnt* pix;
    RowEnt* rows;
    int2* ext;
    int32_t* tile_count;
    int4* chunks;
    int4* tiles;
    int32_t B, N, P, apl, cap_tiles;
    int64_t Ppad;
};
int sparse_tail_min_pixels(int N);
hipError_t launch_sparse_tail_rows(const SparseTailArgs& a, hipStream_t s);
hipError_t launch_joint_entropy_rank(const PostCfg& c, const PostBuffers& b, hipStream_t s);
hipError_t launch_validation_post(const PostCfg& c, const PostBuffers& b, hipStream_t s);

struct NmsArgs {
    int32_t B, A;
    const int32_t* num_kept;
    const float* corners;
    const float* ranking;
    float* work_scores;
    int32_t* work_begin;
    int32_t* selected;
    int32_t* num_selected;
    int32_t max_out;
    float iou_thr, sigma;
    int32_t variant;
};
hipError_t launch_nms(const NmsArgs& a, hipStream_t s);

struct ClusterArgs {
    int32_t B, A, C, max_out;
    const int32_t* num_kept;
    const int32_t* selected;
    const int32_t* num_selected;
    const float* corners;
    const float* counts;
    const float* means;
    const float* covs;
    float thr;
    const float* affinity; int32_t affinity_img;
    float* out_scores; float* out_means; float* out_covs; float* out_counts;
};
hipError_t launch_cluster_fuse(const ClusterArgs& a, hipStream_t s);
hipError_t launch_iou_matrix(const float* corners, int M, float* out, hipStream_t s);
hipError_t launch_pack_records(const int32_t* num, const float* scores, const float* means, const float* covs, const float* counts,
                               float* rec, int B, int K, int C, hipStream_t s);

struct PreprocArgs {
    const uint8_t* src;
    float* dst;
    int32_t B, sh, sw;
    int32_t rh, rw;
    int32_t H, W;
    int32_t crop_y, crop_x, pad_y, pad_x, vis_h, vis_w;
    int32_t resize;
    float scale_y, scale_x;
    float mean[3];
};
hipError_t launch_preprocess(const PreprocArgs& a, hipStream_t s);

struct LossArgs {
    int32_t B, A, C;
    int32_t do_cls;
    int32_t reg_kind;
    float label_smoothing;
    const float* cls; const float* cls_t;
    const float* box; const float* box_t;
    const float* cov;
    const float* anchors;
    const uint8_t* pos; const uint8_t* neg;
};
hipError_t launch_loss(const LossArgs& a, float* partial, int nblocks, hipStream_t s);
hipError_t launch_loss_reduce(const float* partial, int nblocks, float* sums4, hipStream_t s);
hipError_t launch_loss_backward(const LossArgs& a, const float* sums4, float w_cls, float w_reg, float* dcls, float* dbox, float* dcov,
                                hipStream_t s);

bool conv_pointwise_eligible(const ConvArgs& a);
bool conv_pointwise_can_fuse_next(const ConvArgs& a);
bool conv_pointwise_can_fuse_dual(const ConvArgs& a);
hipError_t launch_conv_pointwise(const ConvArgs& a, hipStream_t s);
bool conv_slide3x3_eligible(const ConvArgs& a);
hipError_t launch_conv_slide3x3(const ConvArgs& a, hipStream_t s);

hipError_t launch_gather_transpose(const void* in, const RowEnt* rows, void* out, int M, int Kpad, int C, int cstride,
                                   int taps, int KW, bool append_ones_row, hipStream_t s, bool f32 = false);
hipError_t launch_fill_row_bf16(void* row, int n_set, int n_total, float value, hipStream_t s);

struct FoldArgs {
    const float* kernel;
    const float* bias;
    const float *gamma, *beta, *mean, *var;
    float eps;
    int32_t taps, cin, cout, cout_pad;
    uint16_t* w_fwd;
    float* w_fwd32;
    uint16_t* w_bwd;
    uint16_t* w_flip;
    float* b_fwd;
    int32_t f32;
};
struct ActBwdArgs {
    const float* dout;
    const uint16_t* out_bf16;
    const RowEnt* rows;
    float* dres;
    uint16_t* dz;
    uint16_t* dzp;
    uint16_t* dzt;
    int32_t M, cout, cout_pad, out_cstride, res_cstride, Kpad;
    float scale;
    int32_t f32;
};
struct UnfoldArgs {
    const float* dwp;
    const float* kernel; const float* bias;
    const float *gamma, *mean, *var;
    float eps;
    int32_t taps, cin, cout;
    float *d_kernel, *d_bias, *d_gamma, *d_beta;
    float* dot;
    float l2;
    float* l2_loss;
};
hipError_t launch_fold_pack(const FoldArgs& a, hipStream_t s);
hipError_t launch_fold_pack_all(const FoldArgs* device_array, int count, long max_elems, hipStream_t s);
hipError_t launch_act_backward_gather(const ActBwdArgs& a, hipStream_t s, bool* wrote_transpose = nullptr);
hipError_t launch_relu_merge(const float* dout_relu, const void* out, float* dout, long n, hipStream_t s, bool f32 = false);
hipError_t launch_col2im(const float* dxcol, const RowEnt* rows, float* din, int M, int taps, int KW, int cin, int in_cstride, hipStream_t s);
hipError_t launch_stem_pool_backward(const void* stem_out, const float* dpool, void* dz, int B, int ih, int iw, int oh, int ow, int pool_pitch,
                                     int pool_plane, hipStream_t s, bool f32 = false);
hipError_t launch_unfold_grad(const UnfoldArgs& a, hipStream_t s);
hipError_t launch_l2_grad(const float* w, float* g, long n, float rate, float* loss_acc, hipStream_t s);
hipError_t launch_sumsq(const float* g, long n, float* acc, float* partial1024, hipStream_t s);
hipError_t launch_adam(float* w, const float* g, float* m, float* v, long n, const float* sumsq, float clip, const float* lr_t, float beta1, float beta2,
                       float eps, hipStream_t s);
hipError_t launch_f32_to_bf16(const float* in, void* out, long n, hipStream_t s);
hipError_t launch_make_dgrad_rows(const RowEnt* fwd, RowEnt* out, int M, hipStream_t s);
```

### bayes-od-rc_amd/csrc/post_kernels.hip

```cpp
#include "kernels.h"
#include "philox.h"
#include <algorithm>
#include <math.h>

#define POST_BLOCK 256
#define MAXC 16

struct Mat4 { float m[4][4]; };

__device__ __forceinline__ Mat4 inv_spd4_once(const Mat4& a) {
    float g[4][4];
#pragma unroll
    for (int i = 0; i < 4; ++i)
#pragma unroll
        for (int j = 0; j < 4; ++j) g[i][j] = 0.f;
#pragma unroll
    for (int j = 0; j < 4; ++j) {
        float d = a.m[j][j];
#pragma unroll
        for (int k = 0; k < j; ++k) d -= g[j][k] * g[j][k];
        const float dj = sqrtf(d);
        g[j][j] = dj;
        const float inv = 1.0f / dj;
#pragma unroll
// ... 331 lines not shown
    for (int i = 0; i < 4; ++i) { out20[i] = mu[i] + best; for (int j = 0; j < 4; ++j) out20[4 + i * 4 + j] = lik.m[i][j]; }
    return;
#endif
    Mat4 pcov;
    float pm[4];
    if (c.gaussian_iso) {
        const Mat4 prec = inv_spd4(lik);
        const float pp = 1.0f / c.iso_var;
        Mat4 post_prec = prec;
#pragma unroll
        for (int i = 0; i < 4; ++i) post_prec.m[i][i] += pp;
        pcov = inv_spd4(post_prec);
        const float am[4] = {anc.x, anc.y, anc.z, anc.w};
        float inter[4];
#pragma unroll
        for (int i = 0; i < 4; ++i) {
            float s = 0.f;
#pragma unroll
            for (int k = 0; k < 4; ++k) s += prec.m[i][k] * mu[k];
            inter[i] = pp * am[i] + s;
        }
#pragma unroll
        for (int i = 0; i < 4; ++i) {
            float s = 0.f;
#pragma unroll
            for (int k = 0; k < 4; ++k) s += pcov.m[i][k] * inter[k];
            pm[i] = s;
        }
    } else {
        pcov = lik;
#pragma unroll
        for (int i = 0; i < 4; ++i) pm[i] = mu[i];
    }
    if (c.kitti_sh > 0.f) {
        const float sc[4] = {c.kitti_sh, c.kitti_sw, c.kitti_sh, c.kitti_sw};
#pragma unroll
        for (int i = 0; i < 4; ++i) {
            pm[i] *= sc[i];
#pragma unroll
            for (int j = 0; j < 4; ++j) pcov.m[i][j] = sc[i] * pcov.m[i][j] * sc[j];
        }
    }
#if !(defined(BOD_POST_SELFCHECK) && BOD_POST_SELFCHECK == 2)
#pragma unroll
    for (int i = 0; i < 4; ++i) {
        pb.means[o * 4 + i] = pm[i];
#pragma unroll
        for (int j = 0; j < 4; ++j) pb.covs[o * 16 + i * 4 + j] = pcov.m[i][j];
    }
#endif
#if defined(BOD_POST_SELFCHECK)
#pragma unroll
    for (int i = 0; i < 4; ++i) {
        out20[i] = pm[i];
#pragma unroll
        for (int j = 0; j < 4; ++j) out20[4 + i * 4 + j] = pcov.m[i][j];
    }
#endif
#if defined(BOD_POST_SELFCHECK) && BOD_POST_SELFCHECK == 2
    out20[0] += best * 0.f;
    return;
#else
    pb.ranking[o] = best;
    pb.corners[o * 4 + 0] = pm[0] - pm[2] / 2.0f;
    pb.corners[o * 4 + 1] = pm[1] - pm[3] / 2.0f;
    pb.corners[o * 4 + 2] = pm[0] + pm[2] / 2.0f;
    pb.corners[o * 4 + 3] = pm[1] + pm[3] / 2.0f;
#endif
}

#define POST_FUSE_BLOCKS 8
template <int C>
__global__ __launch_bounds__(POST_BLOCK) void post_fuse_kernel(PostCfg c, PostBuffers pb, int nblocks) {
    const int b = blockIdx.y;
    const int m = pb.num_kept[b];
#if defined(BOD_POST_SELFCHECK)
    for (int slot = blockIdx.x * POST_BLOCK + threadIdx.x; slot < m; slot += gridDim.x * POST_BLOCK) {
        float r1[20], r2[20];
#if BOD_POST_SELFCHECK == 2
        FuseIn fin;
        {
            const size_t o = (size_t)b * c.A + slot;
            const int a = pb.anchor_index[o];
            fin.anc = reinterpret_cast<const float4*>(pb.anchors)[a];
            for (int q = 0; q < 4; ++q) fin.ab[q] = (reinterpret_cast<const float4*>(pb.agg_box) + ((size_t)b * c.A + a) * 4)[q];
            for (int q = 0; q < 5; ++q) fin.cv[q] = reinterpret_cast<const float2*>(pb.agg_cov + ((size_t)b * c.A + a) * 10)[q];
            for (int q = 0; q < 8; ++q) fin.dc[q] = q < C ? pb.d_counts[((size_t)b * c.A + a) * C + q] : 0.f;
        }
        asm volatile("s_waitcnt vmcnt(0) lgkmcnt(0)" ::: "memory");
        post_fuse_anchor<C>(c, pb, b, slot, r1, fin);
        post_fuse_anchor<C>(c, pb, b, slot, r2, fin);
#else
        post_fuse_anchor<C>(c, pb, b, slot, r1);
        post_fuse_anchor<C>(c, pb, b, slot, r2);
#endif
        if ((threadIdx.x & 63) == 0) atomicAdd(&g_selfcheck_waves, 1ull);
        int bad = -1;
        for (int i = 19; i >= 0; --i) if (__float_as_uint(r1[i]) != __float_as_uint(r2[i])) bad = i;
        if (bad >= 0) {
            const unsigned int k = atomicAdd(&g_selfcheck_count, 1u);
            if (k < 4096u) {
                SelfcheckRec r;
                r.hw_id = __builtin_amdgcn_s_getreg((31 << 11) | 4);
                r.xcc_id = __builtin_amdgcn_s_getreg((31 << 11) | 20);
                r.image = (uint32_t)b; r.slot = (uint32_t)slot; r.lane = threadIdx.x & 63; r.elem = (uint32_t)bad;
                r.first = r1[bad]; r.second = r2[bad];
                g_selfcheck_recs[k] = r;
            }
        }
    }
#else
    for (int slot = blockIdx.x * POST_BLOCK + threadIdx.x; slot < m; slot += gridDim.x * POST_BLOCK) post_fuse_anchor<C>(c, pb, b, slot);
#endif
}
#if defined(BOD_POST_SELFCHECK)
extern "C" int bod_debug_selfcheck_read(unsigned int* count, unsigned long long* waves, void* recs, int max) {
    unsigned int n = 0;
    if (hipMemcpyFromSymbol(&n, HIP_SYMBOL(g_selfcheck_count), 4) != hipSuccess) return 1;
    if (hipMemcpyFromSymbol(waves, HIP_SYMBOL(g_selfcheck_waves), 8) != hipSuccess) return 1;
    const unsigned int m = n < (unsigned)max ? n : (unsigned)max;
    if (m && hipMemcpyFromSymbol(recs, HIP_SYMBOL(g_selfcheck_recs), (size_t)(m < 4096u ? m : 4096u) * sizeof(SelfcheckRec)) != hipSuccess) return 1;
    const unsigned int z = 0; const unsigned long long z8 = 0;
    if (hipMemcpyToSymbol(HIP_SYMBOL(g_selfcheck_count), &z, 4) != hipSuccess || hipMemcpyToSymbol(HIP_SYMBOL(g_selfcheck_waves), &z8, 8) != hipSuccess) return 1;
    *count = n;
    return 0;
}
#endif

hipError_t launch_posterior_keep(const PostCfg& c, const PostBuffers& b, hipStream_t s) {
    const int nblocks = (c.A + POST_BLOCK - 1) / POST_BLOCK;
    dim3 grid(nblocks, c.B);
    if (c.C == 8) hipLaunchKernelGGL(post_sample_kernel<8>, grid, dim3(POST_BLOCK), 0, s, c, b, nblocks);
    else if (c.C == 4) hipLaunchKernelGGL(post_sample_kernel<4>, grid, dim3(POST_BLOCK), 0, s, c, b, nblocks);
    else return hipErrorInvalidValue;
    hipLaunchKernelGGL(post_scan_kernel, dim3(c.B), dim3(POST_BLOCK), 0, s, b, nblocks);
    return hipGetLastError();
}

hipError_t launch_posterior_fuse(const PostCfg& c, const PostBuffers& b, hipStream_t s) {
    const int nblocks = (c.A + POST_BLOCK - 1) / POST_BLOCK;
    dim3 grid(nblocks, c.B);
    if (c.C != 8 && c.C != 4) return hipErrorInvalidValue;
    hipLaunchKernelGGL(post_compact_kernel, grid, dim3(POST_BLOCK), 0, s, c, b, nblocks);
    if (c.C == 8) hipLaunchKernelGGL(post_fuse_kernel<8>, dim3(std::min(nblocks, POST_FUSE_BLOCKS), c.B), dim3(POST_BLOCK), 0, s, c, b, nblocks);
    else hipLaunchKernelGGL(post_fuse_kernel<4>, dim3(std::min(nblocks, POST_FUSE_BLOCKS), c.B), dim3(POST_BLOCK), 0, s, c, b, nblocks);
    return hipGetLastError();
}

hipError_t launch_posterior(const PostCfg& c, const PostBuffers& b, hipStream_t s) {
    const hipError_t e = launch_posterior_keep(c, b, s);
    return e != hipSuccess ? e : launch_posterior_fuse(c, b, s);
}

int sparse_tail_min_pixels(int N) {
    const int Qmax = 256 / N;
    return std::max(1, std::min(Qmax, (XR_EXT_ROWS - 3 * N) / (3 * N) + 1));
}

__device__ __forceinline__ RowEnt sparse_tail_ent(const SparseTailArgs& a, int b, int n, int p) {
    RowEnt e = a.pix[p];
    const int32_t plane = (int32_t)(((int64_t)b * a.N + n) * a.Ppad);
    e.in_off += plane;
    e.out_off += plane;
    e.rng_zs = n | (b << 16);
    e.pad0 = (int32_t)(((int64_t)b * a.N + n) * a.P + p);
    return e;
}

__global__ __launch_bounds__(256) void sparse_tail_rows_kernel(SparseTailArgs a) {
    extern __shared__ uint8_t s_flag[];
    __shared__ int s_nchunk, s_ntile, s_base;
    const int b = blockIdx.x, tid = threadIdx.x, N = a.N, P = a.P;
    const uint8_t* keep = a.keep + (size_t)b * P * a.apl;
    for (int p = tid; p < P; p += blockDim.x) {
        uint8_t f = 0;
        for (int k = 0; k < a.apl; ++k) f |= keep[(size_t)p * a.apl + k];
        s_flag[p] = f ? 1 : 0;
    }
    __syncthreads();
    int4* chunks = a.chunks + (size_t)b * P;
    int4* tiles = a.tiles + (size_t)b * P;
    if (tid == 0) {
        const int Qmax = 256 / N;
        auto adjacent = [&](int p) { return a.pix[p].in_off == a.pix[p - 1].in_off + 1 && a.pix[p].in_pitch == a.pix[p - 1].in_pitch; };
        int nchunk = 0, ntile = 0, Q = 0, X = 0, first = 0;
        bool open = false;
        auto close_tile = [&]() { tiles[ntile++] = make_int4(first, Q, X, 0); open = false; };
        int p = 0;
        while (p < P) {
            if (!s_flag[p]) { ++p; continue; }
            int L = 1;
            while (p + L < P && adjacent(p + L) &&
                   (s_flag[p + L] || (p + L + 1 < P && s_flag[p + L + 1] && adjacent(p + L + 1)))) ++L;
            while (L > 0) {
                if (!open) { first = p; Q = 0; X = 0; open = true; }
                const int take = min(min(L, Qmax - Q), (XR_EXT_ROWS - X) / N - 2);
                if (take < 1) { close_tile(); continue; }
                chunks[nchunk++] = make_int4(p, ntile, Q, X | (take << 16));
                X += N * (take + 2); Q += take; p += take; L -= take;
                if (Q == Qmax) close_tile();
            }
        }
        if (open) close_tile();
        s_nchunk = nchunk; s_ntile = ntile;
        s_base = atomicAdd(a.tile_count, ntile);
    }
    __syncthreads();
    const int nchunk = s_nchunk, ntile = s_ntile, base = s_base;
    if (base + ntile > a.cap_tiles) return;
    for (int i = tid; i < nchunk * N; i += blockDim.x) {
        const int ci = i / N, n = i - ci * N;
        const int4 c = chunks[ci];
        const int p0 = c.x, t = base + c.y, Q0 = c.z, X0 = c.w & 0xFFFF, take = c.w >> 16;
        const int x0 = X0 + n * (take + 2);
        const RowEnt first = sparse_tail_ent(a, b, n, p0);
        int2* ext = a.ext + (size_t)t * XR_EXT_ROWS + x0;
        for (int k = 0; k < take + 2; ++k) ext[k] = make_int2(first.in_off + k, first.in_pitch);
        RowEnt* rows = a.rows + (size_t)t * 256;
        for (int k = 0; k < take; ++k) {
            RowEnt q = sparse_tail_ent(a, b, n, p0 + k);
            q.pad1 = x0 + k;
            rows[(Q0 + k) * N + n] = q;
        }
    }
    RowEnt invalid = a.pix[0];
    invalid.out_off = -1; invalid.pad0 = 0; invalid.pad1 = 0;
    for (int i = tid; i < ntile * 256; i += blockDim.x) {
        const int t = i >> 8, r = i & 255;
        if (r >= tiles[t].y * N) a.rows[(size_t)(base + t) * 256 + r] = invalid;
    }
    for (int i = tid; i < ntile * XR_EXT_ROWS; i += blockDim.x) {
        const int t = i / XR_EXT_ROWS, r = i - t * XR_EXT_ROWS;
        const int4 ti = tiles[t];
        if (r >= ti.z) {
            const RowEnt first = sparse_tail_ent(a, b, 0, ti.x);
            a.ext[(size_t)(base + t) * XR_EXT_ROWS + r] = make_int2(first.in_off, first.in_pitch);
        }
    }
}

hipError_t launch_sparse_tail_rows(const SparseTailArgs& a, hipStream_t s) {
    if (a.B <= 0 || a.P <= 0 || a.N < 1 || 256 / a.N < 1 || XR_EXT_ROWS / a.N - 2 < 1 || a.P > 65536) return hipErrorInvalidValue;
    hipError_t e = hipMemsetAsync(a.tile_count, 0, sizeof(int32_t), s);
    if (e != hipSuccess) return e;
    hipLaunchKernelGGL(sparse_tail_rows_kernel, dim3(a.B), dim3(256), (size_t)a.P, s, a);
    return hipGetLastError();
}

template <int C>
__global__ __launch_bounds__(POST_BLOCK) void val_flag_kernel(PostCfg c, PostBuffers pb, int nblocks) {
    const int a = blockIdx.x * POST_BLOCK + threadIdx.x;
    const int b = blockIdx.y;
    bool keep = false;
    if (a < c.A) {
        const float* l = pb.cls + (((size_t)b * c.N) * c.A + a) * C;
        float v[C];
#pragma unroll
        for (int j = 0; j < C; ++j) v[j] = l[j];
        float mx = v[0];
#pragma unroll
        for (int j = 1; j < C; ++j) mx = fmaxf(mx, v[j]);
        float s = 0.f;
#pragma unroll
        for (int j = 0; j < C; ++j) { v[j] = expf(v[j] - mx); s += v[j]; }
        int best = 0; float bestp = v[0] / s;
        float* dc = pb.d_counts + ((size_t)b * c.A + a) * C;
#pragma unroll
        for (int j = 0; j < C; ++j) {
            const float pj = v[j] / s;
            dc[j] = pj;
            if (j > 0 && pj > bestp) { bestp = pj; best = j; }
        }
        keep = best != C - 1;
        pb.keep[(size_t)b * c.A + a] = keep ? 1 : 0;
    }
    const int n = __syncthreads_count(keep ? 1 : 0);
    if (threadIdx.x == 0) pb.block_counts[(size_t)b * nblocks + blockIdx.x] = n;
}

template <int C>
__global__ __launch_bounds__(POST_BLOCK) void val_fuse_kernel(PostCfg c, PostBuffers pb, int nblocks) {
    __shared__ int wave_off[POST_BLOCK / 64 + 1];
    const int tid = threadIdx.x, lane = tid & 63, wave = tid >> 6;
    const int a = blockIdx.x * POST_BLOCK + tid;
    const int b = blockIdx.y;
    const bool keep = (a < c.A) && pb.keep[(size_t)b * c.A + a];
    const unsigned long long bal = __ballot(keep);
    const int before = __popcll(bal & ((1ull << lane) - 1ull));
    if (lane == 0) wave_off[wave + 1] = __popcll(bal);
    if (tid == 0) wave_off[0] = 0;
    __syncthreads();
    if (tid == 0)
        for (int w = 1; w <= POST_BLOCK / 64; ++w) wave_off[w] += wave_off[w - 1];
    __syncthreads();
    if (!keep) return;
    const int slot = pb.block_counts[(size_t)b * nblocks + blockIdx.x] + wave_off[wave] + before;
    const size_t o = (size_t)b * c.A + slot;
    const float4 anc = reinterpret_cast<const float4*>(pb.anchors)[a];
    const float4 t = reinterpret_cast<const float4*>(pb.box)[((size_t)b * c.N) * c.A + a];
    float bx[4];
    decode_box(anc, t, bx);
    const float* dc = pb.d_counts + ((size_t)b * c.A + a) * C;
    float top = dc[0];
#pragma unroll
    for (int j = 0; j < C; ++j) { pb.counts[o * C + j] = dc[j]; pb.score[o * C + j] = dc[j]; top = fmaxf(top, dc[j]); }
#pragma unroll
    for (int i = 0; i < 4; ++i) pb.means[o * 4 + i] = bx[i];
#pragma unroll
    for (int i = 0; i < 16; ++i) pb.covs[o * 16 + i] = 0.f;
    pb.ranking[o] = top;
    reinterpret_cast<float4*>(pb.corners)[o] = make_float4(bx[0] - bx[2] / 2.0f, bx[1] - bx[3] / 2.0f, bx[0] + bx[2] / 2.0f, bx[1] + bx[3] / 2.0f);
    pb.anchor_index[o] = a;
}

hipError_t launch_validation_post(const PostCfg& c, const PostBuffers& b, hipStream_t s) {
    const int nblocks = (c.A + POST_BLOCK - 1) / POST_BLOCK;
    dim3 grid(nblocks, c.B);
    if (c.C == 8) {
        hipLaunchKernelGGL(val_flag_kernel<8>, grid, dim3(POST_BLOCK), 0, s, c, b, nblocks);
        hipLaunchKernelGGL(post_scan_kernel, dim3(c.B), dim3(POST_BLOCK), 0, s, b, nblocks);
        hipLaunchKernelGGL(val_fuse_kernel<8>, grid, dim3(POST_BLOCK), 0, s, c, b, nblocks);
    } else if (c.C == 4) {
        hipLaunchKernelGGL(val_flag_kernel<4>, grid, dim3(POST_BLOCK), 0, s, c, b, nblocks);
        hipLaunchKernelGGL(post_scan_kernel, dim3(c.B), dim3(POST_BLOCK), 0, s, b, nblocks);
        hipLaunchKernelGGL(val_fuse_kernel<4>, grid, dim3(POST_BLOCK), 0, s, c, b, nblocks);
    } else {
        return hipErrorInvalidValue;
    }
    return hipGetLastError();
}

__device__ __forceinline__ double logdet4_spd(const float* m) {
    double L[4][4];
    double ld = 0.0;
#pragma unroll
    for (int i = 0; i < 4; ++i) {
#pragma unroll
        for (int j = 0; j <= i; ++j) {
            double s = (double)m[i * 4 + j];
#pragma unroll
            for (int k = 0; k < j; ++k) s -= L[i][k] * L[j][k];
            if (i == j) { L[i][i] = sqrt(s); ld += log(s); }
            else L[i][j] = s / L[j][j];
        }
    }
    return ld;
}

__global__ __launch_bounds__(POST_BLOCK) void joint_entropy_kernel(PostCfg c, PostBuffers pb) {
    __shared__ float red[4][POST_BLOCK];
    const int b = blockIdx.x, tid = threadIdx.x;
    const int M = pb.num_kept[b];
    const float two_pi_term = 2.0f + 2.0f * logf(2.0f * 3.14159265358979323846f);
    const float iv = c.iso_var;
    const float prior_ent = two_pi_term + 0.5f * logf(iv * iv * iv * iv);
    const float cat_prior = logf((float)c.C);
    float gmin = INFINITY, gmax = -INFINITY, cmin = INFINITY, cmax = -INFINITY;
    for (int m = tid; m < M; m += POST_BLOCK) {
        const size_t o = (size_t)b * c.A + m;
        const float g = (float)((double)prior_ent - ((double)two_pi_term + 0.5 * logdet4_spd(pb.covs + o * 16)));
        float ce = 0.f;
        for (int j = 0; j < c.C; ++j) { const float p = pb.score[o * c.C + j]; ce -= p * logf(p); }
        const float cg = cat_prior - ce;
        gmin = fminf(gmin, g); gmax = fmaxf(gmax, g);
        cmin = fminf(cmin, cg); cmax = fmaxf(cmax, cg);
    }
    red[0][tid] = gmin; red[1][tid] = gmax; red[2][tid] = cmin; red[3][tid] = cmax;
    __syncthreads();
    for (int s = POST_BLOCK / 2; s > 0; s >>= 1) {
        if (tid < s) {
            red[0][tid] = fminf(red[0][tid], red[0][tid + s]);
            red[1][tid] = fmaxf(red[1][tid], red[1][tid + s]);
            red[2][tid] = fminf(red[2][tid], red[2][tid + s]);
            red[3][tid] = fmaxf(red[3][tid], red[3][tid + s]);
        }
        __syncthreads();
    }
    gmin = red[0][0]; gmax = red[1][0]; cmin = red[2][0]; cmax = red[3][0];
    const float gden = fmaxf(1.0f, gmax - gmin), cden = fmaxf(0.001f, cmax - cmin);
    for (int m = tid; m < M; m += POST_BLOCK) {
        const size_t o = (size_t)b * c.A + m;
        const float g = (float)((double)prior_ent - ((double)two_pi_term + 0.5 * logdet4_spd(pb.covs + o * 16)));
        float ce = 0.f;
        for (int j = 0; j < c.C; ++j) { const float p = pb.score[o * c.C + j]; ce -= p * logf(p); }
        const float cg = cat_prior - ce;
        pb.ranking[o] = (cg - cmin) / cden + (g - gmin) / gden;
    }
}

hipError_t launch_joint_entropy_rank(const PostCfg& c, const PostBuffers& b, hipStream_t s) {
    hipLaunchKernelGGL(joint_entropy_kernel, dim3(c.B), dim3(POST_BLOCK), 0, s, c, b);
    return hipGetLastError();
}

#define NMS_LDS_CAP 6144
#define NMS_MAX_OUT 512
// ... 434 lines not shown
```

### bayes-od-rc_amd/engine.py

```python
import ctypes as C

import numpy as np

from . import _lib
from ._lib import BodConfig, BodSizes, as_f32, fptr, iptr

_KINDS = {"kernel": 0, "bias": 1, "gamma": 2, "beta": 3, "mean": 4, "var": 5}
PRECISIONS = {"bf16": 0, "fp32": 1, "bf16x3": 2, "f16mx": 3, "f16mx4": 4}


def make_config(image_hw, batch=1, mc_samples=10, num_classes=8, anchors_per_location=9, device=0,
                dropout_rate=0.3, use_full_covar=True, bayes_od_config=None, nms_config=None,
                has_covar_head=True, dataset_name='bdd', orig_size=None, nms_variant='A',
                num_categorical_draws=30, layers=(3, 4, 5, 6, 7), precision='bf16', mc_sample_base=0,
                mc_ensemble_size=0, training=False, backbone_depth=50, pipeline_overlap=False):
    bo = bayes_od_config or {'ranking_method': 'score', 'dirichlet_prior': {'type': 'non_informative'},
                             'gaussian_prior': {'type': 'isotropic', 'isotropic_variance': 100000.0}}
    nms = nms_config or {'max_output_size': 100, 'iou_threshold': 0.5, 'soft_nms_sigma': 0.5}
    cfg = BodConfig()
    cfg.device = int(device)
    cfg.image_h, cfg.image_w = int(image_hw[0]), int(image_hw[1])
    cfg.batch, cfg.mc_samples = int(batch), int(mc_samples)
    cfg.num_classes = int(num_classes)
    cfg.anchors_per_location = int(anchors_per_location)
# ... 202 lines not shown
        u8 = C.POINTER(C.c_uint8)
        if images is None:
            ptr, on_dev = self.lib.bod_device_images(self.h), 1
        else:
            img = self._img(images)
            ptr, on_dev = img.ctypes.data, 0
        self._chk(self.lib.bod_train_step(self.h, ptr, on_dev, fptr(ct), fptr(bt), pm.ctypes.data_as(u8), nm.ctypes.data_as(u8),
                                          seed, first_image_id, int(reg_kind), float(label_smoothing), float(w_cls), float(w_reg),
                                          float(l2_rate), float(learning_rate), int(bool(apply_update)), out))
        keys = ("total_loss", "cls_loss", "reg_loss", "covariance_loss", "regularization_loss", "grad_norm")
        return dict(zip(keys, [out[i] for i in range(6)]))

    def train_gradients_view(self):
        import torch
        from .distributed import DeviceArray
        ptr, n = C.c_void_p(), C.c_int64()
        self._chk(self.lib.bod_train_gradients(self.h, C.byref(ptr), C.byref(n)))
        return torch.as_tensor(DeviceArray(ptr.value, (n.value,), "<f4"), device=torch.device("cuda", self.cfg.device))

    def train_apply(self, learning_rate):
        g = C.c_double()
        self._chk(self.lib.bod_train_apply(self.h, float(learning_rate), C.byref(g)))
        return g.value

    def train_get(self, layer, kind, shape, what="value"):
        kinds = {"kernel": 0, "bias": 1, "gamma": 2, "beta": 3}
        whats = {"value": 0, "grad": 1, "adam_m": 2, "adam_v": 3}
        out = np.empty(shape, np.float32)
        self._chk(self.lib.bod_train_get(self.h, layer.encode(), kinds[kind], whats[what], fptr(out), out.size))
        return out

    def train_set_moment(self, layer, kind, what, value):
        kinds = {"kernel": 0, "bias": 1, "gamma": 2, "beta": 3}
        whats = {"adam_m": 2, "adam_v": 3}
        a = as_f32(value)
        self._chk(self.lib.bod_train_set(self.h, layer.encode(), kinds[kind], whats[what], fptr(a), a.size))

    def train_step_count(self, set_to=None):
        got = C.c_int64(0)
        self._chk(self.lib.bod_train_step_count(self.h, C.byref(got), -1 if set_to is None else int(set_to)))
        return int(got.value)

    def validation_post(self):
        self._chk(self.lib.bod_validation_post(self.h))

    def num_kept(self):
        out = np.zeros(self.B, np.int32)
        self._chk(self.lib.bod_get_num_kept(self.h, iptr(out)))
        return out

    def get_posterior(self, image_index=0):
        m = int(self.num_kept()[image_index])
        counts = np.empty((m, self.Ccls), np.float32)
        score = np.empty((m, self.Ccls), np.float32)
        means = np.empty((m, 4), np.float32)
        covs = np.empty((m, 4, 4), np.float32)
        ranking = np.empty((m,), np.float32)
        aidx = np.empty((m,), np.int32)
        self._chk(self.lib.bod_get_posterior(self.h, image_index, fptr(counts), fptr(score), fptr(means),
                                             fptr(covs), fptr(ranking), iptr(aidx)))
        return {"counts": counts, "score": score, "means": means, "covs": covs, "ranking": ranking,
                "anchor_index": aidx}

    def set_posterior(self, image_index, counts, means, covs, ranking):
        counts, means, covs, ranking = as_f32(counts), as_f32(means).reshape(-1, 4), as_f32(covs), as_f32(ranking)
        m = means.shape[0]
        self._chk(self.lib.bod_set_posterior(self.h, image_index, m, fptr(counts), fptr(means), fptr(covs),
                                             fptr(ranking)))

    def nms(self):
        self._chk(self.lib.bod_nms(self.h))

    def get_nms(self, image_index=0):
        idx = np.zeros(self.K, np.int32)
        n = C.c_int32(0)
        self._chk(self.lib.bod_get_nms(self.h, image_index, iptr(idx), C.byref(n)))
        return idx[:n.value].copy()

    def _set_centres(self, image_index, centres):
        c = np.ascontiguousarray(centres, dtype=np.int32)
        self._chk(self.lib.bod_set_nms(self.h, image_index, iptr(c), c.shape[0]))

    def set_affinity(self, image_index, centre_columns):
        c = as_f32(centre_columns)
        self._chk(self.lib.bod_set_affinity(self.h, image_index, fptr(c), c.shape[0], c.shape[1]))

    def get_iou_matrix(self, image_index=0):
        m = int(self.num_kept()[image_index])
        out = np.empty((m, m), np.float32)
        if m:
            self._chk(self.lib.bod_get_iou_matrix(self.h, image_index, fptr(out)))
        return out

    def cluster_fuse(self):
        self._chk(self.lib.bod_cluster_fuse(self.h))

    def get_detections(self, image_index=0):
        k = self.K
        scores = np.empty((k, self.Ccls), np.float32)
        means = np.empty((k, 4), np.float32)
        covs = np.empty((k, 4, 4), np.float32)
        counts = np.empty((k, self.Ccls), np.float32)
        n = C.c_int32(0)
        self._chk(self.lib.bod_get_detections(self.h, image_index, C.byref(n), fptr(scores), fptr(means),
                                              fptr(covs), fptr(counts)))
        n = n.value
        return scores[:n].copy(), means[:n].copy(), covs[:n].copy(), counts[:n].copy()

    def get_detections_batch(self, out=None):
        b, k, c = self.B, self.K, self.Ccls
        if out is None:
            out = {"num": np.empty(b, np.int32), "scores": np.empty((b, k, c), np.float32),
                   "means": np.empty((b, k, 4), np.float32), "covs": np.empty((b, k, 4, 4), np.float32),
                   "counts": np.empty((b, k, c), np.float32)}
        self._chk(self.lib.bod_get_detections_batch(self.h, iptr(out["num"]), fptr(out["scores"]),
                                                    fptr(out["means"]), fptr(out["covs"]), fptr(out["counts"])))
        return out

    def wait_slot(self, slot):
        self._chk(self.lib.bod_collect(self.h, slot, None, None, None, None, None))

    def device_raw_pointers(self, mark_ready=False):
        ptrs = (C.c_void_p * 3)()
        self._chk(self.lib.bod_device_raw(self.h, ptrs, int(mark_ready)))
        return [ptrs[i] for i in range(3)]

    def device_detection_pointers(self, slot=0):
        ptrs = (C.c_void_p * 5)()
        self._chk(self.lib.bod_device_detections(self.h, slot, ptrs))
        b, k, c = self.B, self.K, self.Ccls
        shapes = [(b,), (b, k, c), (b, k, 4), (b, k, 16), (b, k, c)]
        names = ["num", "scores", "means", "covs", "counts"]
        return {n: (int(p), s) for n, p, s in zip(names, ptrs, shapes)}

    def bench_head_conv(self, layer=1, variant=0, iters=10):
        ms, fl = C.c_double(0), C.c_double(0)
        self._chk(self.lib.bod_bench_head_conv(self.h, layer, variant, iters, C.byref(ms), C.byref(fl)))
        return ms.value, fl.value

    def gather_detections(self, slot=-1, comm=None, world=1, rank=0, root=0, want_host=True):
        w = int(self.lib.bod_record_width(self.h))
        out = None
        dev = C.c_void_p(0)
        if rank == root and want_host:
            out = np.empty((world, self.B, self.K, w), np.float32)
        self._chk(self.lib.bod_gather_detections(self.h, int(slot), C.c_void_p(int(comm) if comm else 0), int(world), int(rank), int(root),
                                                 out.ctypes.data if out is not None else None,
                                                 C.byref(dev) if rank == root else None))
        if rank == root and not want_host:
            return int(dev.value or 0), (world, self.B, self.K, w)
        return out

    def plan_info(self):
        info = (C.c_int32 * 8)()
        self._chk(self.lib.bod_plan_info(self.h, info))
        return {"aggregating": bool(info[0]), "fused_head_outputs": bool(info[1]), "row_reuse": bool(info[2]),
                "fan_out_row_reuse": bool(info[3]), "ops": int(info[4]), "plane_row_reuse_layers": int(info[5]), "tower_mx": bool(info[6]), "tower_mx_format": int(info[6]),
                "sparse_tail": bool(info[7])}

    @property
    def aggregating(self):
        return self.plan_info()["aggregating"]

    def profile_begin(self, which=None):
        if which is not None:
            self._chk(self.lib.bod_profile_select(self.h, int(which)))
        self._chk(self.lib.bod_profile_begin(self.h))

    def profile_end(self):
        hm, pm, fl = C.c_double(0), C.c_double(0), C.c_double(0)
        hl, pl = C.c_int64(0), C.c_int64(0)
        self._chk(self.lib.bod_profile_end(self.h, C.byref(hm), C.byref(hl), C.byref(fl), C.byref(pm), C.byref(pl)))
        return {"head_conv_ms": hm.value, "head_conv_launches": hl.value, "head_conv_flops": fl.value,
                "posterior_ms": pm.value, "posterior_launches": pl.value}


def stage_conv(x, w, bias=None, stride=1, padding="same", relu=False, residual=None, dropout_rate=0.0,
               seed=0, layer_id=0, image_id=0, round_output_bf16=False, device=0, precision='bf16'):
    lib = _lib.load()
    x, w = as_f32(x), as_f32(w)
    b, h, wd, cin = x.shape
    kh, kw, cin2, cout = w.shape
    if cin2 != cin:
        raise ValueError("kernel Cin %d != input Cin %d" % (cin2, cin))
    if padding == "same":
        oh, ow = -(-h // stride), -(-wd // stride)
    else:
        oh, ow = (h - kh) // stride + 1, (wd - kw) // stride + 1
    out = np.empty((b, oh, ow, cout), np.float32)
    bias = as_f32(bias) if bias is not None else None
    residual = as_f32(residual) if residual is not None else None
    st = lib.bod_stage_conv(device, fptr(x), b, h, wd, cin, fptr(w), fptr(bias), kh, kw, cout, stride,
                            int(padding == "same"), int(relu), fptr(residual), float(dropout_rate), seed,
                            layer_id, image_id, int(round_output_bf16), PRECISIONS[precision], fptr(out))
    _lib.check(lib, None, st)
    return out


def stage_conv_wgrad(x, dy, kernel_hw, stride=1, padding="same", ksplit=0, device=0):
    lib = _lib.load()
    x, dy = as_f32(x), as_f32(dy)
    b, h, wd, cin = x.shape
    kh, kw = int(kernel_hw[0]), int(kernel_hw[1])
    cout = dy.shape[-1]
    dw = np.empty((kh, kw, cin, cout), np.float32)
    db = np.empty((cout,), np.float32)
    st = lib.bod_stage_conv_wgrad(device, fptr(x), b, h, wd, cin, fptr(dy), kh, kw, cout, stride,
                                  int(padding == "same"), int(ksplit), fptr(dw), fptr(db))
    _lib.check(lib, None, st)
    return dw, db


def stage_conv_dgrad(dy, w, padding="same", device=0):
    w = as_f32(w)
    if padding != "same" or w.shape[0] % 2 == 0 or w.shape[1] % 2 == 0:
        raise ValueError("stage_conv_dgrad covers stride-1 SAME convolutions with odd kernels")
    wt = np.ascontiguousarray(np.transpose(w[::-1, ::-1], (0, 1, 3, 2)))
    return stage_conv(dy, wt, None, stride=1, padding="same", device=device)
```

### include/bayesod.h

```cpp
#ifndef BAYESOD_H
#define BAYESOD_H

#include <stdint.h>

#ifdef __cplusplus
extern "C" {
#endif

typedef struct bod_context* bod_handle;

typedef enum {
    BOD_OK = 0,
    BOD_ERR_INVALID_ARG = 1,
    BOD_ERR_HIP = 2,
    BOD_ERR_OOM = 3,
    BOD_ERR_NOT_READY = 4,
    BOD_ERR_NO_DEVICE = 5
} bod_status;

enum { BOD_RANK_SCORE = 0, BOD_RANK_JOINT_ENTROPY = 1 };
enum { BOD_NMS_VARIANT_A = 0, BOD_NMS_VARIANT_B = 1 };
enum { BOD_HEAD_CLS = 0, BOD_HEAD_REG = 1, BOD_HEAD_COV = 2 };
enum { BOD_PRECISION_BF16 = 0, BOD_PRECISION_FP32 = 1, BOD_PRECISION_BF16X3 = 2, BOD_PRECISION_F16MX = 3, BOD_PRECISION_F16MX4 = 4 };

typedef struct {
    int32_t device;
    int32_t image_h, image_w;
    int32_t batch;
    int32_t mc_samples;
    int32_t num_classes;
    int32_t anchors_per_location;
    int32_t min_level, max_level;
    float   dropout_rate;
    int32_t use_full_covar;
    int32_t dirichlet_non_informative;
    int32_t gaussian_isotropic;
    float   isotropic_variance;
    int32_t ranking_method;
    int32_t nms_max_output_size;
    float   nms_iou_threshold;
    float   nms_soft_sigma;
    int32_t nms_variant;
    int32_t num_categorical_draws;
    int32_t has_covar_head;
    float   kitti_scale_h, kitti_scale_w;
    int32_t precision;
    int32_t mc_sample_base;
    int32_t mc_ensemble_size;
    int32_t training;
    int32_t backbone_depth;
    int32_t pipeline_overlap;
    int32_t reserved[2];
} bod_config;

typedef struct {
    int32_t num_pixels;
    int32_t num_anchors;
    int32_t level_h[8], level_w[8];
    int32_t num_levels;
    int32_t max_detections;
    int64_t device_bytes;
} bod_sizes;

const char* bod_version(void);
const char* bod_last_error(bod_handle h);

bod_status bod_create(const bod_config* cfg, bod_handle* out);
bod_status bod_destroy(bod_handle h);
bod_status bod_query_sizes(bod_handle h, bod_sizes* out);
bod_status bod_update_config(bod_handle h, const bod_config* cfg);

bod_status bod_load_weight(bod_handle h, const char* name, int32_t kind,
                           const int64_t* shape, int32_t ndim, const float* data);
bod_status bod_finalize_weights(bod_handle h);

bod_status bod_set_anchors(bod_handle h, const float* anchors_vuhw, int32_t num_anchors);

bod_status bod_forward(bod_handle h, const float* images, int32_t images_on_device,
                       uint64_t seed, uint32_t first_image_id);
bod_status bod_get_raw(bod_handle h, float* cls, float* box, float* covar_params);
bod_status bod_set_raw(bod_handle h, const float* cls, const float* box, const float* covar_params);
bod_status bod_get_pyramid(bod_handle h, int32_t level_index, float* out);

bod_status bod_posterior(bod_handle h, uint64_t seed, uint32_t first_image_id);
bod_status bod_validation_post(bod_handle h);
bod_status bod_get_num_kept(bod_handle h, int32_t* num_kept);
bod_status bod_get_posterior(bod_handle h, int32_t image_index, float* counts, float* score,
                             float* means, float* covs, float* ranking, int32_t* anchor_index);
bod_status bod_set_posterior(bod_handle h, int32_t image_index, int32_t m, const float* counts,
                             const float* means, const float* covs, const float* ranking);

bod_status bod_nms(bod_handle h);
bod_status bod_get_nms(bod_handle h, int32_t image_index, int32_t* indices, int32_t* num_selected);
bod_status bod_set_nms(bod_handle h, int32_t image_index, const int32_t* indices, int32_t num_selected);
bod_status bod_get_iou_matrix(bod_handle h, int32_t image_index, float* iou);

bod_status bod_cluster_fuse(bod_handle h);
bod_status bod_set_affinity(bod_handle h, int32_t image_index, const float* centre_columns, int32_t k, int32_t m);
bod_status bod_get_detections(bod_handle h, int32_t image_index, int32_t* num_detections,
                              float* scores, float* means, float* covs, float* counts);

bod_status bod_get_detections_batch(bod_handle h, int32_t* num_detections, float* scores, float* means,
                                    float* covs, float* counts);
bod_status bod_device_detections(bod_handle h, int32_t slot, void** ptrs5);
bod_status bod_device_raw(bod_handle h, void** ptrs3, int32_t mark_ready);

bod_status bod_infer(bod_handle h, const float* images, int32_t images_on_device,
                     uint64_t seed, uint32_t first_image_id);

bod_status bod_infer_async(bod_handle h, const float* images, int32_t images_on_device,
                           uint64_t seed, uint32_t first_image_id, int32_t* slot);
bod_status bod_collect(bod_handle h, int32_t slot, int32_t* num_detections, float* scores,
                       float* means, float* covs, float* counts);

bod_status bod_upload_images(bod_handle h, const float* host_images);
bod_status bod_upload_frames_u8(bod_handle h, const uint8_t* rgb, int32_t src_h, int32_t src_w,
                                const float* rgb_means, int32_t aspect_resize);
bod_status bod_upload_frames_u8_async(bod_handle h, const uint8_t* rgb, int32_t src_h, int32_t src_w,
                                      const float* rgb_means, int32_t aspect_resize, int32_t buffer);
const float* bod_device_images_buffer(bod_handle h, int32_t buffer);
const float* bod_device_images(bod_handle h);
bod_status bod_synchronize(bod_handle h);

bod_status bod_stage_conv(int32_t device, const float* x, int32_t B, int32_t H, int32_t W, int32_t Cin,
                          const float* w, const float* bias, int32_t KH, int32_t KW, int32_t Cout,
                          int32_t stride, int32_t same_padding, int32_t relu, const float* residual,
                          float dropout_rate, uint64_t seed, int32_t layer_id, uint32_t image_id,
                          int32_t round_output_bf16, int32_t precision, float* out);

bod_status bod_stage_conv_wgrad(int32_t device, const float* x, int32_t B, int32_t H, int32_t W, int32_t Cin,
                                const float* dy, int32_t KH, int32_t KW, int32_t Cout, int32_t stride,
                                int32_t same_padding, int32_t ksplit, float* dw, float* db);

bod_status bod_train_step(bod_handle h, const float* images, int32_t images_on_device, const float* cls_targets,
                          const float* box_targets, const uint8_t* positive_mask, const uint8_t* negative_mask,
                          uint64_t seed, uint32_t first_image_id, int32_t reg_kind, float label_smoothing,
                          float w_cls, float w_reg, float l2_rate, float learning_rate, int32_t apply_update,
                          double* out6);
bod_status bod_train_gradients(bod_handle h, void** device_ptr, int64_t* count);
bod_status bod_train_apply(bod_handle h, float learning_rate, double* grad_norm);
bod_status bod_train_get(bod_handle h, const char* layer, int32_t kind, int32_t what, float* out, int64_t n);
bod_status bod_train_set(bod_handle h, const char* layer, int32_t kind, int32_t what, const float* data, int64_t n);
bod_status bod_train_step_count(bod_handle h, int64_t* get, int64_t set);

bod_status bod_loss_forward(int32_t device, int32_t B, int32_t A, int32_t C, const float* cls,
                            const float* cls_targets, const float* box, const float* box_targets,
                            const float* covar_params, const float* anchors, const uint8_t* positive_mask,
                            const uint8_t* negative_mask, int32_t do_classification, int32_t reg_kind,
                            float label_smoothing, double* out4);

bod_status bod_loss_backward(int32_t device, int32_t B, int32_t A, int32_t C, const float* cls,
                             const float* cls_targets, const float* box, const float* box_targets,
                             const float* covar_params, const float* anchors, const uint8_t* positive_mask,
                             const uint8_t* negative_mask, int32_t do_cls, int32_t reg_kind, float label_smoothing,
                             float w_cls, float w_reg, double* out4, float* dcls, float* dbox, float* dcov);

bod_status bod_bench_head_conv(bod_handle h, int32_t layer, int32_t variant, int32_t iters,
                               double* mean_ms, double* flops_per_launch);

bod_status bod_profile_begin(bod_handle h);
bod_status bod_profile_select(bod_handle h, int32_t which);
bod_status bod_profile_end(bod_handle h, double* head_conv_ms, int64_t* head_conv_launches,
                           double* head_conv_flops, double* posterior_ms, int64_t* posterior_launches);

int32_t bod_record_width(bod_handle h);
bod_status bod_gather_detections(bod_handle h, int32_t slot, void* nccl_comm, int32_t world, int32_t rank, int32_t root,
                                 float* gathered_host, float** gathered_device);

bod_status bod_plan_info(bod_handle h, int32_t* info8);

#ifdef __cplusplus
}
#endif
#endif
```

### include/bayesod_cdef.h

```cpp
typedef struct bod_context* bod_handle;
typedef enum {
    BOD_OK = 0,
    BOD_ERR_INVALID_ARG = 1,
    BOD_ERR_HIP = 2,
    BOD_ERR_OOM = 3,
    BOD_ERR_NOT_READY = 4,
    BOD_ERR_NO_DEVICE = 5
} bod_status;
enum { BOD_RANK_SCORE = 0, BOD_RANK_JOINT_ENTROPY = 1 };
enum { BOD_NMS_VARIANT_A = 0, BOD_NMS_VARIANT_B = 1 };
enum { BOD_HEAD_CLS = 0, BOD_HEAD_REG = 1, BOD_HEAD_COV = 2 };
enum { BOD_PRECISION_BF16 = 0, BOD_PRECISION_FP32 = 1, BOD_PRECISION_BF16X3 = 2, BOD_PRECISION_F16MX = 3, BOD_PRECISION_F16MX4 = 4 };
typedef struct {
    int32_t device;
    int32_t image_h, image_w;
    int32_t batch;
    int32_t mc_samples;
    int32_t num_classes;
    int32_t anchors_per_location;
    int32_t min_level, max_level;
    float   dropout_rate;
    int32_t use_full_covar;
    int32_t dirichlet_non_informative;
    int32_t gaussian_isotropic;
    float   isotropic_variance;
    int32_t ranking_method;
    int32_t nms_max_output_size;
    float   nms_iou_threshold;
    float   nms_soft_sigma;
    int32_t nms_variant;
    int32_t num_categorical_draws;
    int32_t has_covar_head;
    float   kitti_scale_h, kitti_scale_w;
    int32_t precision;
    int32_t mc_sample_base;
    int32_t mc_ensemble_size;
    int32_t training;
    int32_t backbone_depth;
    int32_t pipeline_overlap;
    int32_t reserved[2];
} bod_config;
typedef struct {
    int32_t num_pixels;
    int32_t num_anchors;
    int32_t level_h[8], level_w[8];
    int32_t num_levels;
    int32_t max_detections;
    int64_t device_bytes;
} bod_sizes;
const char* bod_version(void);
const char* bod_last_error(bod_handle h);
bod_status bod_create(const bod_config* cfg, bod_handle* out);
bod_status bod_destroy(bod_handle h);
bod_status bod_query_sizes(bod_handle h, bod_sizes* out);
bod_status bod_update_config(bod_handle h, const bod_config* cfg);
bod_status bod_load_weight(bod_handle h, const char* name, int32_t kind,
                           const int64_t* shape, int32_t ndim, const float* data);
bod_status bod_finalize_weights(bod_handle h);
bod_status bod_set_anchors(bod_handle h, const float* anchors_vuhw, int32_t num_anchors);
bod_status bod_forward(bod_handle h, const float* images, int32_t images_on_device,
                       uint64_t seed, uint32_t first_image_id);
bod_status bod_get_raw(bod_handle h, float* cls, float* box, float* covar_params);
bod_status bod_set_raw(bod_handle h, const float* cls, const float* box, const float* covar_params);
bod_status bod_get_pyramid(bod_handle h, int32_t level_index, float* out);
bod_status bod_posterior(bod_handle h, uint64_t seed, uint32_t first_image_id);
bod_status bod_validation_post(bod_handle h);
bod_status bod_get_num_kept(bod_handle h, int32_t* num_kept);
bod_status bod_get_posterior(bod_handle h, int32_t image_index, float* counts, float* score,
                             float* means, float* covs, float* ranking, int32_t* anchor_index);
bod_status bod_set_posterior(bod_handle h, int32_t image_index, int32_t m, const float* counts,
                             const float* means, const float* covs, const float* ranking);
bod_status bod_nms(bod_handle h);
bod_status bod_get_nms(bod_handle h, int32_t image_index, int32_t* indices, int32_t* num_selected);
bod_status bod_set_nms(bod_handle h, int32_t image_index, const int32_t* indices, int32_t num_selected);
bod_status bod_get_iou_matrix(bod_handle h, int32_t image_index, float* iou);
bod_status bod_cluster_fuse(bod_handle h);
bod_status bod_set_affinity(bod_handle h, int32_t image_index, const float* centre_columns, int32_t k, int32_t m);
bod_status bod_get_detections(bod_handle h, int32_t image_index, int32_t* num_detections,
                              float* scores, float* means, float* covs, float* counts);
bod_status bod_get_detections_batch(bod_handle h, int32_t* num_detections, float* scores, float* means,
                                    float* covs, float* counts);
bod_status bod_device_detections(bod_handle h, int32_t slot, void** ptrs5);
bod_status bod_device_raw(bod_handle h, void** ptrs3, int32_t mark_ready);
bod_status bod_infer(bod_handle h, const float* images, int32_t images_on_device,
                     uint64_t seed, uint32_t first_image_id);
bod_status bod_infer_async(bod_handle h, const float* images, int32_t images_on_device,
                           uint64_t seed, uint32_t first_image_id, int32_t* slot);
bod_status bod_collect(bod_handle h, int32_t slot, int32_t* num_detections, float* scores,
                       float* means, float* covs, float* counts);
bod_status bod_upload_images(bod_handle h, const float* host_images);
bod_status bod_upload_frames_u8(bod_handle h, const uint8_t* rgb, int32_t src_h, int32_t src_w,
                                const float* rgb_means, int32_t aspect_resize);
bod_status bod_upload_frames_u8_async(bod_handle h, const uint8_t* rgb, int32_t src_h, int32_t src_w,
                                      const float* rgb_means, int32_t aspect_resize, int32_t buffer);
const float* bod_device_images_buffer(bod_handle h, int32_t buffer);
const float* bod_device_images(bod_handle h);
bod_status bod_synchronize(bod_handle h);
bod_status bod_stage_conv(int32_t device, const float* x, int32_t B, int32_t H, int32_t W, int32_t Cin,
                          const float* w, const float* bias, int32_t KH, int32_t KW, int32_t Cout,
                          int32_t stride, int32_t same_padding, int32_t relu, const float* residual,
                          float dropout_rate, uint64_t seed, int32_t layer_id, uint32_t image_id,
                          int32_t round_output_bf16, int32_t precision, float* out);
bod_status bod_stage_conv_wgrad(int32_t device, const float* x, int32_t B, int32_t H, int32_t W, int32_t Cin,
                                const float* dy, int32_t KH, int32_t KW, int32_t Cout, int32_t stride,
                                int32_t same_padding, int32_t ksplit, float* dw, float* db);
bod_status bod_train_step(bod_handle h, const float* images, int32_t images_on_device, const float* cls_targets,
                          const float* box_targets, const uint8_t* positive_mask, const uint8_t* negative_mask,
                          uint64_t seed, uint32_t first_image_id, int32_t reg_kind, float label_smoothing,
                          float w_cls, float w_reg, float l2_rate, float learning_rate, int32_t apply_update,
                          double* out6);
bod_status bod_train_gradients(bod_handle h, void** device_ptr, int64_t* count);
bod_status bod_train_apply(bod_handle h, float learning_rate, double* grad_norm);
bod_status bod_train_get(bod_handle h, const char* layer, int32_t kind, int32_t what, float* out, int64_t n);
bod_status bod_train_set(bod_handle h, const char* layer, int32_t kind, int32_t what, const float* data, int64_t n);
bod_status bod_train_step_count(bod_handle h, int64_t* get, int64_t set);
bod_status bod_loss_forward(int32_t device, int32_t B, int32_t A, int32_t C, const float* cls,
                            const float* cls_targets, const float* box, const float* box_targets,
                            const float* covar_params, const float* anchors, const uint8_t* positive_mask,
                            const uint8_t* negative_mask, int32_t do_classification, int32_t reg_kind,
                            float label_smoothing, double* out4);
bod_status bod_loss_backward(int32_t device, int32_t B, int32_t A, int32_t C, const float* cls,
                             const float* cls_targets, const float* box, const float* box_targets,
                             const float* covar_params, const float* anchors, const uint8_t* positive_mask,
                             const uint8_t* negative_mask, int32_t do_cls, int32_t reg_kind, float label_smoothing,
                             float w_cls, float w_reg, double* out4, float* dcls, float* dbox, float* dcov);
bod_status bod_bench_head_conv(bod_handle h, int32_t layer, int32_t variant, int32_t iters,
                               double* mean_ms, double* flops_per_launch);
bod_status bod_profile_begin(bod_handle h);
bod_status bod_profile_select(bod_handle h, int32_t which);
bod_status bod_profile_end(bod_handle h, double* head_conv_ms, int64_t* head_conv_launches,
                           double* head_conv_flops, double* posterior_ms, int64_t* posterior_launches);
int32_t bod_record_width(bod_handle h);
bod_status bod_gather_detections(bod_handle h, int32_t slot, void* nccl_comm, int32_t world, int32_t rank, int32_t root,
                                 float* gathered_host, float** gathered_device);
bod_status bod_plan_info(bod_handle h, int32_t* info8);
```

Measured before the change: 2140 images/sec.

## Compute layer-2 box/covar tower only on halo of kept pixels in sparse tail

Extends the sparse tail so that, at inference, the box and covariance head tower layers 1 and 2 run densely only in a raw/forward variant. In the aggregating path they instead run over a dilated halo of kept pixels, built as a second tile table. The sparse-tail kernel now builds two row/ext tables (tail and halo), using level-aware run packing plus 3x3 dilation in a new shared header. Separate raw-forward and rerun ops are added so raw consumers still get the full result. The aim is to skip dense conv work on anchors later discarded, at the cost of more planning kernel work and extra op variants. Optional stats printing and a plan-info accessor are also added.

```diff
diff --git a/bayes-od-rc_amd/_lib.py b/bayes-od-rc_amd/_lib.py
--- a/bayes-od-rc_amd/_lib.py
+++ b/bayes-od-rc_amd/_lib.py
@@ -104,6 +104,7 @@
     "bod_profile_begin": (C.c_int, [_H]),
     "bod_profile_select": (C.c_int, [_H, C.c_int32]),
     "bod_plan_info": (C.c_int, [_H, C.POINTER(C.c_int32)]),
+    "bod_plan_info_n": (C.c_int, [_H, C.POINTER(C.c_int32), C.c_int32]),
     "bod_record_width": (C.c_int32, [_H]),
     "bod_gather_detections": (C.c_int, [_H, C.c_int32, C.c_void_p, C.c_int32, C.c_int32, C.c_int32, C.c_void_p, C.POINTER(C.c_void_p)]),
     "bod_profile_end": (C.c_int, [_H, C.POINTER(C.c_double), C.POINTER(C.c_int64),
diff --git a/bayes-od-rc_amd/csrc/engine.hip b/bayes-od-rc_amd/csrc/engine.hip
--- a/bayes-od-rc_amd/csrc/engine.hip
+++ b/bayes-od-rc_amd/csrc/engine.hip
@@ -47,6 +47,8 @@
     int flavour = 0;
     int head[3] = {-1, -1, -1};
     bool hx_pyramid = false;
+    enum { ANY_RAW = 0, RAW_FORWARD = 1, RAW_RERUN = 2 };
+    int raw_use = ANY_RAW;
 };
 enum { FLAVOUR_BOTH = 0, FLAVOUR_RAW = 1, FLAVOUR_AGG = 2 };
 
@@ -254,6 +256,8 @@
     bool plan_fused_out = false, plan_xreuse = false, plan_xreuse0 = false;
     bool raw_valid = false, agg_valid = false;
     bool plan_sparse = false;
+    bool plan_halo = false;
+    int dense_plain_tiles = 0;
     SparseTailArgs sparse{};
     bool agg_sparse = false;
     bool keep_ready = false;
@@ -866,6 +870,7 @@
         return BOD_OK;
     };
     if (xreuse) BODCHK(make_xr_tiles(t2, &d2x, &dext, &m2x));
+    h->dense_plain_tiles = m2x / 256;
     RowEnt* d1x = nullptr; int2* dext1 = nullptr; int m1x = 0;
     bool xreuse0 = xreuse;
     if (const char* e = getenv("BOD_FAN_XREUSE")) xreuse0 = xreuse0 && atoi(e) != 0;
@@ -917,10 +922,18 @@
     bool sparse = agg && split_on && h->es == 2 && !h->split && !mx_plan && !c.pipeline_overlap && h->A == h->P * c.anchors_per_location &&
                   h->P <= 65536;
     if (const char* e = getenv("BOD_SPARSE_TAIL")) sparse = sparse && atoi(e) != 0;
+    bool halo = sparse && !train_mode;
+    if (const char* e = getenv("BOD_SPARSE_HALO")) halo = halo && atoi(e) != 0;
     if (sparse) {
         SparseTailArgs& sa = h->sparse;
+        const int tables = halo ? 2 : 1;
         sa.B = B; sa.N = N; sa.P = h->P; sa.apl = c.anchors_per_location; sa.Ppad = h->Ppad;
-        sa.cap_tiles = B * (h->P / sparse_tail_min_pixels(N) + 1);
+        sa.cap_tiles = B * (h->P / st_min_pixels(N) + 1);
+        sa.lv.n = 5;
+        {
+            const PyramidGeometry pg = pyramid_geometry(h->lh, h->lw);
+            for (int l = 0; l < 5; ++l) { sa.lv.lw[l] = pg.lw[l]; sa.lv.lh[l] = pg.lh[l]; sa.lv.p0[l] = (int32_t)pg.lvl_p0[l]; }
+        }
         RowEnt* pix = nullptr;
         BODCHK(h->dalloc(&pix, (size_t)h->P, false));
         HIPCHK(h, hipMemcpyAsync(pix, t2.data(), (size_t)h->P * sizeof(RowEnt), hipMemcpyHostToDevice, h->stream));
@@ -928,13 +941,21 @@
         sa.pix = pix;
         BODCHK(h->dalloc(&sa.rows, (size_t)sa.cap_tiles * 256, false));
         BODCHK(h->dalloc(&sa.ext, (size_t)sa.cap_tiles * XR_EXT_ROWS, false));
-        BODCHK(h->dalloc(&sa.tile_count, 1));
-        BODCHK(h->dalloc(&sa.chunks, (size_t)B * h->P, false));
-        BODCHK(h->dalloc(&sa.tiles, (size_t)B * h->P, false));
+        if (halo) {
+            BODCHK(h->dalloc(&sa.halo_rows, (size_t)sa.cap_tiles * 256, false));
+            BODCHK(h->dalloc(&sa.halo_ext, (size_t)sa.cap_tiles * XR_EXT_ROWS, false));
+        }
+        BODCHK(h->dalloc(&sa.tile_count, 2));
+        BODCHK(h->dalloc(&sa.runs, (size_t)tables * B * h->P, false));
+        BODCHK(h->dalloc(&sa.chunks, (size_t)tables * B * h->P, false));
+        BODCHK(h->dalloc(&sa.tiles, (size_t)tables * B * h->P, false));
     }
     h->plan_sparse = sparse;
+    h->plan_halo = halo;
     Op sparse_op; sparse_op.kind = Op::CONV; sparse_op.is_head3x3 = true; sparse_op.flavour = FLAVOUR_AGG;
     int sparse_groups = 0; PackedConv sparse_pc{};
+    Op halo_op = sparse_op;
+    int halo_groups = 0; PackedConv halo_pc{};
     h->agg_plan = agg; h->plan_fused_out = fuse_out; h->plan_xreuse = xreuse; h->plan_xreuse0 = xreuse0; h->plan_mx = mx_plan ? mxf : 0;
     int hfmt[3] = {mxf, mxf, mxf};
     if (mxf == 2) { const char* e = getenv("BOD_MX4_BOX_HX"); if (e && atoi(e) != 0) hfmt[1] = 1; }
@@ -955,6 +976,9 @@
         Op op; op.kind = Op::CONV; op.is_head3x3 = true; op.flavour = both ? FLAVOUR_BOTH : flav;
         int g = 0; PackedConv pc0{};
         double fused_flops = 0;
+        const bool both_flav = op.flavour == FLAVOUR_BOTH;
+        ConvGroup raw_cg{}; PackedConv raw_pc{}; std::string raw_wname; bool has_raw = false;
+        ConvGroup full_cg[3]{}; std::string full_wname[3]; PackedConv full_pc{}; int nfull = 0;
         for (int hd = 0; hd < nheads; ++hd) {
             if (layer >= kHeadConvs[hd]) continue;
             if (split_launch && (part == 1) != (layer == kHeadConvs[hd] - 1)) continue;
@@ -984,6 +1008,17 @@
                 }
                 fused_flops += 2.0 * ((double)B * N * h->P) * 256.0 * out_ch[hd];
             }
+            if (halo && both_flav && ((layer == 1 && hd == 1) || (layer == 2 && hd == 2))) {
+                halo_op.conv.g[halo_groups] = cg;
+                halo_op.wname[halo_groups] = op.wname[g];
+                if (halo_groups++ == 0) halo_pc = pc;
+                halo_op.flops += 2.0 * ((double)B * N * h->P) * 256.0 * 2304.0;
+                raw_cg = cg; raw_pc = pc; raw_wname = op.wname[g]; has_raw = true;
+                if (nfull == 0) full_pc = pc;
+                full_cg[nfull] = cg; full_wname[nfull++] = op.wname[g];
+                op.wname[g].clear();
+                continue;
+            }
             if (sparse && flav == FLAVOUR_AGG && hd != 0) {
                 sparse_op.conv.g[sparse_groups] = cg;
                 sparse_op.wname[sparse_groups] = op.wname[g];
@@ -996,40 +1031,70 @@
             }
             op.conv.g[g] = cg;
             if (g == 0) pc0 = pc;
+            if (nfull == 0) full_pc = pc;
+            full_cg[nfull] = cg; full_wname[nfull++] = op.wname[g];
             ++g;
         }
-        if (g == 0) continue;
+        if (g == 0 && !has_raw) continue;
         const int M = layer == 0 ? B * h->P : B * N * h->P;
-        ConvArgs a = base_args(pc0, layer == 0 ? d1 : d2, M, 256, 256);
-        for (int q = 0; q < g; ++q) a.g[q] = op.conv.g[q];
-        a.groups = g;
-        a.flags = CONV_RELU | (mc ? CONV_DROPOUT : 0);
-        a.fan_count = layer == 0 ? N : 1;
-        a.fan_stride = (int32_t)h->Ppad;
-        a.drop_threshold = thr; a.drop_scale = dscale;
-        a.mx = mx_plan ? ((layer == 0 && !mx_l0) ? 2 : (lfmt == 2 ? 3 : 1)) : 0;
-        op.hx_pyramid = mx_l0 && layer == 0;
-        {
-            static const int mx_loader = getenv("BOD_MX_LOADER") ? atoi(getenv("BOD_MX_LOADER")) : 1;
-            static const int tower_loader = getenv("BOD_TOWER_LOADER") ? atoi(getenv("BOD_TOWER_LOADER")) : 0;
-            a.mx_loader = mx_plan ? mx_loader : ((h->es == 2 && layer > 0) ? tower_loader : 0);
-        }
-        if (xreuse0 && layer == 0) { a.rows = d1x; a.M = m1x; a.ext = dext1; a.xreuse = 2; }
-        if (xreuse && layer > 0) {
-            a.rows = d2x; a.M = m2x; a.ext = dext;
-            if (agg && layer >= 2 && !(split_launch && part == 0)) { a.rows = d2a; a.M = m2a; a.ext = dexta; }
-            a.xreuse = 2;
-        }
-        op.conv = a;
-        op.flops = 2.0 * M * 256.0 * 2304.0 * g + fused_flops;
-        op.name = "head_tower_layer_" + std::to_string(layer) + (both ? "" : flav == FLAVOUR_AGG ? "(aggregating)" : flav == FLAVOUR_RAW ? "(raw)" : "");
-        op.same_geom = N == 1;
-        h->ops.push_back(op);
+        if (has_raw) op.flavour = FLAVOUR_AGG;
+        for (int twin = 0; twin < 3; ++twin) {
+            if (twin == 0 ? g == 0 : !has_raw) continue;
+            if (twin > 0) {
+                op = Op{}; op.kind = Op::CONV; op.is_head3x3 = true; op.flavour = FLAVOUR_RAW; fused_flops = 0;
+                if (twin == 1) {
+                    for (int q = 0; q < nfull; ++q) { op.conv.g[q] = full_cg[q]; op.wname[q] = full_wname[q]; }
+                    pc0 = full_pc; g = nfull; op.raw_use = Op::RAW_FORWARD;
+                } else {
+                    op.conv.g[0] = raw_cg; op.wname[0] = raw_wname;
+                    pc0 = raw_pc; g = 1; op.raw_use = Op::RAW_RERUN;
+                }
+            }
+            ConvArgs a = base_args(pc0, layer == 0 ? d1 : d2, M, 256, 256);
+            for (int q = 0; q < g; ++q) a.g[q] = op.conv.g[q];
+            a.groups = g;
+            a.flags = CONV_RELU | (mc ? CONV_DROPOUT : 0);
+            a.fan_count = layer == 0 ? N : 1;
+            a.fan_stride = (int32_t)h->Ppad;
+            a.drop_threshold = thr; a.drop_scale = dscale;
+            a.mx = mx_plan ? ((layer == 0 && !mx_l0) ? 2 : (lfmt == 2 ? 3 : 1)) : 0;
+            op.hx_pyramid = mx_l0 && layer == 0;
+            {
+                static const int mx_loader = getenv("BOD_MX_LOADER") ? atoi(getenv("BOD_MX_LOADER")) : 1;
+                static const int tower_loader = getenv("BOD_TOWER_LOADER") ? atoi(getenv("BOD_TOWER_LOADER")) : 0;
+                a.mx_loader = mx_plan ? mx_loader : ((h->es == 2 && layer > 0) ? tower_loader : 0);
+            }
+            if (xreuse0 && layer == 0) { a.rows = d1x; a.M = m1x; a.ext = dext1; a.xreuse = 2; }
+            if (xreuse && layer > 0) {
+                a.rows = d2x; a.M = m2x; a.ext = dext;
+                if (agg && layer >= 2 && !(split_launch && part == 0)) { a.rows = d2a; a.M = m2a; a.ext = dexta; }
+                a.xreuse = 2;
+            }
+            op.conv = a;
+            op.flops = 2.0 * M * 256.0 * 2304.0 * g + fused_flops;
+            op.name = "head_tower_layer_" + std::to_string(layer) + (twin == 1 ? "(raw)" : twin == 2 ? "(rerun)" : has_raw ? "(aggregating)" :
+                      both ? "" : flav == FLAVOUR_AGG ? "(aggregating)" : flav == FLAVOUR_RAW ? "(raw)" : "");
+            op.same_geom = N == 1;
+            h->ops.push_back(op);
+        }
     }
     if (sparse_groups > 0) {
         Op keep; keep.kind = Op::KEEP; keep.flavour = FLAVOUR_AGG; keep.name = "head_tower_layer_3(keep)";
         h->ops.push_back(keep);
         const SparseTailArgs& sa = h->sparse;
+        if (halo_groups > 0) {
+            ConvArgs a = base_args(halo_pc, sa.halo_rows, sa.cap_tiles * 256, 256, 256);
+            for (int q = 0; q < halo_groups; ++q) a.g[q] = halo_op.conv.g[q];
+            a.groups = halo_groups;
+            a.flags = CONV_RELU | (mc ? CONV_DROPOUT : 0);
+            a.fan_count = 1; a.fan_stride = (int32_t)h->Ppad;
+            a.drop_threshold = thr; a.drop_scale = dscale;
+            a.ext = sa.halo_ext; a.xreuse = 2; a.tile_count = sa.tile_count + 1;
+            a.mx_loader = getenv("BOD_TOWER_LOADER") ? atoi(getenv("BOD_TOWER_LOADER")) : 0;
+            halo_op.conv = a;
+            halo_op.name = "head_tower_layer_2(halo)";
+            h->ops.push_back(halo_op);
+        }
         ConvArgs a = base_args(sparse_pc, sa.rows, sa.cap_tiles * 256, 256, 256);
         for (int q = 0; q < sparse_groups; ++q) a.g[q] = sparse_op.conv.g[q];
         a.groups = sparse_groups;
@@ -1139,6 +1204,47 @@
     return p;
 }
 
+bod_status sparse_stats(bod_context* h, hipStream_t st) {
+    const SparseTailArgs& sa = h->sparse;
+    int32_t cnt[2] = {0, 0};
+    std::vector<uint8_t> keep((size_t)sa.B * sa.P * sa.apl);
+    HIPCHK(h, hipMemcpyAsync(cnt, sa.tile_count, sizeof(cnt), hipMemcpyDeviceToHost, st));
+    HIPCHK(h, hipMemcpyAsync(keep.data(), h->pb.keep, keep.size(), hipMemcpyDeviceToHost, st));
+    HIPCHK(h, hipStreamSynchronize(st));
+    const SparseLevels& lv = sa.lv;
+    std::vector<uint8_t> f((size_t)sa.P);
+    std::vector<double> share[3];
+    for (auto& v : share) v.assign(lv.n + 1, 0.0);
+    for (int b = 0; b < sa.B; ++b) {
+        for (int p = 0; p < sa.P; ++p) {
+            uint8_t k = 0;
+            for (int a = 0; a < sa.apl; ++a) k |= keep[((size_t)b * sa.P + p) * sa.apl + a];
+            f[p] = k ? ST_KEPT : 0;
+        }
+        for (int p = 0; p < sa.P; ++p) if (st_member(f.data(), lv, p, ST_KEPT)) f[p] |= ST_TAIL;
+        for (int p = 0; p < sa.P; ++p) if (st_dilated(f.data(), lv, p)) f[p] |= ST_DIL;
+        for (int p = 0; p < sa.P; ++p) if (st_member(f.data(), lv, p, ST_DIL)) f[p] |= ST_HALO;
+        for (int p = 0; p < sa.P; ++p) {
+            int l, y, x;
+            st_level_x(lv, p, l, y, x);
+            const uint8_t bits[3] = {ST_KEPT, ST_TAIL, ST_HALO};
+            for (int t = 0; t < 3; ++t) if (f[p] & bits[t]) { share[t][l] += 1; share[t][lv.n] += 1; }
+        }
+    }
+    fprintf(stderr, "# sparse tables: B %d N %d P %d  tail tiles %d  halo tiles %d  dense plain tiles %d  f = %.4f  tail / dense %.4f\n",
+            sa.B, sa.N, sa.P, cnt[0], cnt[1], h->dense_plain_tiles, (double)cnt[1] / h->dense_plain_tiles, (double)cnt[0] / h->dense_plain_tiles);
+    const char* what[3] = {"kept", "tail", "halo"};
+    for (int t = 0; t < 3; ++t) {
+        fprintf(stderr, "# sparse tables: %s pixel share per level", what[t]);
+        for (int l = 0; l <= lv.n; ++l) {
+            const double pix = l < lv.n ? (double)sa.B * lv.lw[l] * lv.lh[l] : (double)sa.B * sa.P;
+            fprintf(stderr, " %s%.4f", l < lv.n ? "" : "all ", share[t][l] / pix);
+        }
+        fprintf(stderr, "\n");
+    }
+    return BOD_OK;
+}
+
 struct Markers {
     bool on = false;
     int (*push)(const char*) = nullptr;
@@ -1220,6 +1326,7 @@
         hipStream_t st = is_front ? fs : h->stream;
         ++op_i;
         if ((op.flavour != FLAVOUR_BOTH && op.flavour != flavour) || (only_flavoured && op.flavour == FLAVOUR_BOTH)) continue;
+        if (op.raw_use == (only_flavoured ? Op::RAW_FORWARD : Op::RAW_RERUN)) continue;
         if ((int)op_i - 1 < h->dev_op_lo || (int)op_i - 1 >= h->dev_op_hi) continue;
         if (ov && first_back) {
             HIPCHK(h, hipEventRecord(h->ev_front_done[par], fs));
@@ -1260,6 +1367,8 @@
                 sa.keep = h->pb.keep;
                 HIPCHK(h, launch_sparse_tail_rows(sa, st));
                 h->keep_ready = true; h->keep_seed = seed; h->keep_first = first_image;
+                static const bool stats = [] { const char* e = getenv("BOD_SPARSE_STATS"); return e && atoi(e) != 0; }();
+                if (stats) BODCHK(sparse_stats(h, st));
                 break;
             }
             case Op::POOL:
@@ -2664,6 +2773,15 @@
     return BOD_OK;
 }
 
+bod_status bod_plan_info_n(bod_handle h, int32_t* info, int32_t n) {
+    if (!h || !info || n < 0) return BOD_ERR_INVALID_ARG;
+    int32_t all[9];
+    BODCHK(bod_plan_info(h, all));
+    all[8] = h->plan_halo;
+    for (int i = 0; i < n && i < 9; ++i) info[i] = all[i];
+    return BOD_OK;
+}
+
 bod_status bod_profile_select(bod_handle h, int32_t which) {
     if (!h) return BOD_ERR_INVALID_ARG;
     if (which < 0 || which > 2) return h->fail(BOD_ERR_INVALID_ARG, "bod_profile_select: %d", which);
diff --git a/bayes-od-rc_amd/csrc/kernels.h b/bayes-od-rc_amd/csrc/kernels.h
--- a/bayes-od-rc_amd/csrc/kernels.h
+++ b/bayes-od-rc_amd/csrc/kernels.h
@@ -2,6 +2,7 @@
 #include <hip/hip_runtime.h>
 #include <stdint.h>
 #include "plan_tables.h"
+#include "sparse_tables.h"
 
 
 struct ConvGroup {
@@ -132,13 +133,16 @@
     const RowEnt* pix;
     RowEnt* rows;
     int2* ext;
+    RowEnt* halo_rows;
+    int2* halo_ext;
     int32_t* tile_count;
-    int4* chunks;
-    int4* tiles;
+    int2* runs;
+    StQuad* chunks;
+    StQuad* tiles;
     int32_t B, N, P, apl, cap_tiles;
     int64_t Ppad;
-};
-int sparse_tail_min_pixels(int N);
+    SparseLevels lv;
+};
 hipError_t launch_sparse_tail_rows(const SparseTailArgs& a, hipStream_t s);
 hipError_t launch_joint_entropy_rank(const PostCfg& c, const PostBuffers& b, hipStream_t s);
 hipError_t launch_validation_post(const PostCfg& c, const PostBuffers& b, hipStream_t s);
diff --git a/bayes-od-rc_amd/csrc/post_kernels.hip b/bayes-od-rc_amd/csrc/post_kernels.hip
--- a/bayes-od-rc_amd/csrc/post_kernels.hip
+++ b/bayes-od-rc_amd/csrc/post_kernels.hip
@@ -507,96 +507,107 @@
     return e != hipSuccess ? e : launch_posterior_fuse(c, b, s);
 }
 
-int sparse_tail_min_pixels(int N) {
-    const int Qmax = 256 / N;
-    return std::max(1, std::min(Qmax, (XR_EXT_ROWS - 3 * N) / (3 * N) + 1));
-}
-
-__device__ __forceinline__ RowEnt sparse_tail_ent(const SparseTailArgs& a, int b, int n, int p) {
-    RowEnt e = a.pix[p];
-    const int32_t plane = (int32_t)(((int64_t)b * a.N + n) * a.Ppad);
-    e.in_off += plane;
-    e.out_off += plane;
-    e.rng_zs = n | (b << 16);
-    e.pad0 = (int32_t)(((int64_t)b * a.N + n) * a.P + p);
-    return e;
-}
-
 __global__ __launch_bounds__(256) void sparse_tail_rows_kernel(SparseTailArgs a) {
     extern __shared__ uint8_t s_flag[];
-    __shared__ int s_nchunk, s_ntile, s_base;
-    const int b = blockIdx.x, tid = threadIdx.x, N = a.N, P = a.P;
+    __shared__ int s_cnt[2][256];
+    __shared__ int s_nrun[2], s_nchunk[2], s_ntile[2], s_base[2];
+    const int b = blockIdx.x, tid = threadIdx.x, N = a.N, P = a.P, B = a.B;
+    const int T = a.halo_rows ? 2 : 1;
+    const SparseLevels& lv = a.lv;
     const uint8_t* keep = a.keep + (size_t)b * P * a.apl;
     for (int p = tid; p < P; p += blockDim.x) {
         uint8_t f = 0;
         for (int k = 0; k < a.apl; ++k) f |= keep[(size_t)p * a.apl + k];
-        s_flag[p] = f ? 1 : 0;
-    }
-    __syncthreads();
-    int4* chunks = a.chunks + (size_t)b * P;
-    int4* tiles = a.tiles + (size_t)b * P;
-    if (tid == 0) {
-        const int Qmax = 256 / N;
-        auto adjacent = [&](int p) { return a.pix[p].in_off == a.pix[p - 1].in_off + 1 && a.pix[p].in_pitch == a.pix[p - 1].in_pitch; };
-        int nchunk = 0, ntile = 0, Q = 0, X = 0, first = 0;
-        bool open = false;
-        auto close_tile = [&]() { tiles[ntile++] = make_int4(first, Q, X, 0); open = false; };
-        int p = 0;
-        while (p < P) {
-            if (!s_flag[p]) { ++p; continue; }
-            int L = 1;
-            while (p + L < P && adjacent(p + L) &&
-                   (s_flag[p + L] || (p + L + 1 < P && s_flag[p + L + 1] && adjacent(p + L + 1)))) ++L;
-            while (L > 0) {
-                if (!open) { first = p; Q = 0; X = 0; open = true; }
-                const int take = min(min(L, Qmax - Q), (XR_EXT_ROWS - X) / N - 2);
-                if (take < 1) { close_tile(); continue; }
-                chunks[nchunk++] = make_int4(p, ntile, Q, X | (take << 16));
-                X += N * (take + 2); Q += take; p += take; L -= take;
-                if (Q == Qmax) close_tile();
+        s_flag[p] = f ? ST_KEPT : 0;
+    }
+    __syncthreads();
+    for (int p = tid; p < P; p += blockDim.x) if (st_member(s_flag, lv, p, ST_KEPT)) s_flag[p] |= ST_TAIL;
+    if (T == 2) {
+        __syncthreads();
+        for (int p = tid; p < P; p += blockDim.x) if (st_dilated(s_flag, lv, p)) s_flag[p] |= ST_DIL;
+        __syncthreads();
+        for (int p = tid; p < P; p += blockDim.x) if (st_member(s_flag, lv, p, ST_DIL)) s_flag[p] |= ST_HALO;
+    }
+    __syncthreads();
+    const int share = (P + 255) / 256, q0 = min(P, tid * share), q1 = min(P, q0 + share);
+    int cnt[2] = {0, 0};
+    for (int t = 0; t < T; ++t) {
+        const uint8_t bit = t == 0 ? ST_TAIL : ST_HALO;
+        for (int p = q0; p < q1; ++p) cnt[t] += st_run_edge(s_flag, lv, p, bit) & 1;
+        s_cnt[t][tid] = cnt[t];
+    }
+    __syncthreads();
+    for (int d = 1; d < 256; d <<= 1) {
+        int v[2] = {0, 0};
+        for (int t = 0; t < T; ++t) v[t] = tid >= d ? s_cnt[t][tid - d] : 0;
+        __syncthreads();
+        for (int t = 0; t < T; ++t) s_cnt[t][tid] += v[t];
+        __syncthreads();
+    }
+    for (int t = 0; t < T; ++t) {
+        const uint8_t bit = t == 0 ? ST_TAIL : ST_HALO;
+        int2* runs = a.runs + ((size_t)t * B + b) * P;
+        int r = s_cnt[t][tid] - cnt[t];
+        for (int p = q0; p < q1; ++p) {
+            const int edge = st_run_edge(s_flag, lv, p, bit);
+            if (edge & 1) runs[r++].x = p;
+            if (edge & 2) runs[r - 1].y = p;
+        }
+        if (tid == 255) s_nrun[t] = s_cnt[t][255];
+    }
+    __syncthreads();
+    const int wave = tid >> 6, lane = tid & 63;
+    if (wave < T) {
+        const int t = wave;
+        const int2* runs = a.runs + ((size_t)t * B + b) * P;
+        StQuad* chunks = a.chunks + ((size_t)t * B + b) * P;
+        StQuad* tiles = a.tiles + ((size_t)t * B + b) * P;
+        const int nrun = s_nrun[t];
+        StPack st{0, 0, 0, 0, 0, 0};
+        for (int r0 = 0; r0 < nrun; r0 += 64) {
+            const int2 mine = r0 + lane < nrun ? runs[r0 + lane] : make_int2(0, 0);
+            const int n = min(64, nrun - r0);
+            for (int j = 0; j < n; ++j) {
+                const int p = __shfl(mine.x, j), q = __shfl(mine.y, j);
+                st_pack_run(st, p, q - p + 1, N, chunks, tiles, lane == 0);
             }
         }
-        if (open) close_tile();
-        s_nchunk = nchunk; s_ntile = ntile;
-        s_base = atomicAdd(a.tile_count, ntile);
-    }
-    __syncthreads();
-    const int nchunk = s_nchunk, ntile = s_ntile, base = s_base;
-    if (base + ntile > a.cap_tiles) return;
-    for (int i = tid; i < nchunk * N; i += blockDim.x) {
-        const int ci = i / N, n = i - ci * N;
-        const int4 c = chunks[ci];
-        const int p0 = c.x, t = base + c.y, Q0 = c.z, X0 = c.w & 0xFFFF, take = c.w >> 16;
-        const int x0 = X0 + n * (take + 2);
-        const RowEnt first = sparse_tail_ent(a, b, n, p0);
-        int2* ext = a.ext + (size_t)t * XR_EXT_ROWS + x0;
-        for (int k = 0; k < take + 2; ++k) ext[k] = make_int2(first.in_off + k, first.in_pitch);
-        RowEnt* rows = a.rows + (size_t)t * 256;
-        for (int k = 0; k < take; ++k) {
-            RowEnt q = sparse_tail_ent(a, b, n, p0 + k);
-            q.pad1 = x0 + k;
-            rows[(Q0 + k) * N + n] = q;
-        }
-    }
-    RowEnt invalid = a.pix[0];
-    invalid.out_off = -1; invalid.pad0 = 0; invalid.pad1 = 0;
-    for (int i = tid; i < ntile * 256; i += blockDim.x) {
-        const int t = i >> 8, r = i & 255;
-        if (r >= tiles[t].y * N) a.rows[(size_t)(base + t) * 256 + r] = invalid;
-    }
-    for (int i = tid; i < ntile * XR_EXT_ROWS; i += blockDim.x) {
-        const int t = i / XR_EXT_ROWS, r = i - t * XR_EXT_ROWS;
-        const int4 ti = tiles[t];
-        if (r >= ti.z) {
-            const RowEnt first = sparse_tail_ent(a, b, 0, ti.x);
-            a.ext[(size_t)(base + t) * XR_EXT_ROWS + r] = make_int2(first.in_off, first.in_pitch);
+        st_pack_close(st, tiles, lane == 0);
+        if (lane == 0) {
+            s_nchunk[t] = st.nchunk; s_ntile[t] = st.ntile;
+            s_base[t] = atomicAdd(a.tile_count + t, st.ntile);
+        }
+    }
+    __syncthreads();
+    const RowEnt invalid = st_invalid_row(a.pix[0]);
+    for (int t = 0; t < T; ++t) {
+        const int nchunk = s_nchunk[t], ntile = s_ntile[t], base = s_base[t];
+        if (base + ntile > a.cap_tiles) continue;
+        RowEnt* rows = t == 0 ? a.rows : a.halo_rows;
+        ExtRow* ext = reinterpret_cast<ExtRow*>(t == 0 ? a.ext : a.halo_ext);
+        const StQuad* chunks = a.chunks + ((size_t)t * B + b) * P;
+        const StQuad* tiles = a.tiles + ((size_t)t * B + b) * P;
+        for (int i = tid; i < nchunk * N; i += blockDim.x) {
+            const int ci = i / N, n = i - ci * N;
+            const StQuad c = chunks[ci];
+            st_write_piece(c, n, b, base + c.y, a.pix, N, P, a.Ppad, rows, ext);
+        }
+        for (int i = tid; i < ntile * 256; i += blockDim.x) {
+            const int tt = i >> 8, r = i & 255;
+            if (st_pad_row(tiles[tt], r, N)) rows[(size_t)(base + tt) * 256 + r] = invalid;
+        }
+        for (int i = tid; i < ntile * XR_EXT_ROWS; i += blockDim.x) {
+            const int tt = i / XR_EXT_ROWS, r = i - tt * XR_EXT_ROWS;
+            const StQuad ti = tiles[tt];
+            if (r >= ti.z) ext[(size_t)(base + tt) * XR_EXT_ROWS + r] = st_pad_ext(ti, b, a.pix, N, P, a.Ppad);
         }
     }
 }
 
 hipError_t launch_sparse_tail_rows(const SparseTailArgs& a, hipStream_t s) {
-    if (a.B <= 0 || a.P <= 0 || a.N < 1 || 256 / a.N < 1 || XR_EXT_ROWS / a.N - 2 < 1 || a.P > 65536) return hipErrorInvalidValue;
-    hipError_t e = hipMemsetAsync(a.tile_count, 0, sizeof(int32_t), s);
+    if (a.B <= 0 || a.P <= 0 || a.N < 1 || 256 / a.N < 1 || XR_EXT_ROWS / a.N - 2 < 1 || a.P > 65536 || a.lv.n < 1 || a.lv.n > 5)
+        return hipErrorInvalidValue;
+    hipError_t e = hipMemsetAsync(a.tile_count, 0, 2 * sizeof(int32_t), s);
     if (e != hipSuccess) return e;
     hipLaunchKernelGGL(sparse_tail_rows_kernel, dim3(a.B), dim3(256), (size_t)a.P, s, a);
     return hipGetLastError();
diff --git a/bayes-od-rc_amd/csrc/sparse_tables.h b/bayes-od-rc_amd/csrc/sparse_tables.h
--- /dev/null
+++ b/bayes-od-rc_amd/csrc/sparse_tables.h
@@ -0,0 +1,126 @@
+#pragma once
+#include "plan_tables.h"
+
+#if defined(__HIPCC__) || defined(__HIP__)
+#define ST_HD __host__ __device__
+#else
+#define ST_HD
+#endif
+
+enum : uint8_t { ST_KEPT = 1, ST_TAIL = 2, ST_DIL = 4, ST_HALO = 8 };
+
+struct SparseLevels {
+    int32_t n;
+    int32_t lw[5], lh[5];
+    int32_t p0[5];
+};
+
+struct alignas(16) StQuad { int32_t x, y, z, w; };
+
+struct StPack { int32_t Q, X, first, open, nchunk, ntile; };
+
+ST_HD inline void st_level_x(const SparseLevels& g, int p, int& l, int& y, int& x) {
+    l = 0;
+    while (l + 1 < g.n && p >= g.p0[l + 1]) ++l;
+    const int q = p - g.p0[l];
+    y = q / g.lw[l];
+    x = q - y * g.lw[l];
+}
+
+ST_HD inline bool st_member(const uint8_t* f, const SparseLevels& g, int p, uint8_t bit) {
+    if (f[p] & bit) return true;
+    int l, y, x;
+    st_level_x(g, p, l, y, x);
+    return x > 0 && x + 1 < g.lw[l] && (f[p - 1] & bit) && (f[p + 1] & bit);
+}
+
+ST_HD inline bool st_dilated(const uint8_t* f, const SparseLevels& g, int p) {
+    int l, y, x;
+    st_level_x(g, p, l, y, x);
+    for (int dy = -1; dy <= 1; ++dy) {
+        const int yy = y + dy;
+        if (yy < 0 || yy >= g.lh[l]) continue;
+        for (int dx = -1; dx <= 1; ++dx) {
+            const int xx = x + dx;
+            if (xx < 0 || xx >= g.lw[l]) continue;
+            if (f[g.p0[l] + yy * g.lw[l] + xx] & ST_TAIL) return true;
+        }
+    }
+    return false;
+}
+
+ST_HD inline int st_run_edge(const uint8_t* f, const SparseLevels& g, int p, uint8_t bit) {
+    if (!(f[p] & bit)) return 0;
+    int l, y, x;
+    st_level_x(g, p, l, y, x);
+    return ((x == 0 || !(f[p - 1] & bit)) ? 1 : 0) | ((x + 1 == g.lw[l] || !(f[p + 1] & bit)) ? 2 : 0);
+}
+
+ST_HD inline void st_pack_run(StPack& s, int p, int L, int N, StQuad* chunks, StQuad* tiles, bool write) {
+    const int Qmax = 256 / N;
+    while (L > 0) {
+        if (!s.open) { s.first = p; s.Q = 0; s.X = 0; s.open = 1; }
+        int take = L < Qmax - s.Q ? L : Qmax - s.Q;
+        const int room = (XR_EXT_ROWS - s.X) / N - 2;
+        take = take < room ? take : room;
+        if (take < 1) {
+            if (write) tiles[s.ntile] = StQuad{s.first, s.Q, s.X, 0};
+            ++s.ntile; s.open = 0;
+            continue;
+        }
+        if (write) chunks[s.nchunk] = StQuad{p, s.ntile, s.Q, s.X | (take << 16)};
+        ++s.nchunk;
+        s.X += N * (take + 2); s.Q += take; p += take; L -= take;
+        if (s.Q == Qmax) {
+            if (write) tiles[s.ntile] = StQuad{s.first, s.Q, s.X, 0};
+            ++s.ntile; s.open = 0;
+        }
+    }
+}
+
+ST_HD inline void st_pack_close(StPack& s, StQuad* tiles, bool write) {
+    if (!s.open) return;
+    if (write) tiles[s.ntile] = StQuad{s.first, s.Q, s.X, 0};
+    ++s.ntile; s.open = 0;
+}
+
+ST_HD inline RowEnt st_row(const RowEnt& pix_p, int b, int n, int p, int N, int P, int64_t Ppad) {
+    RowEnt e = pix_p;
+    const int32_t plane = (int32_t)(((int64_t)b * N + n) * Ppad);
+    e.in_off += plane;
+    e.out_off += plane;
+    e.rng_zs = n | (b << 16);
+    e.pad0 = (int32_t)(((int64_t)b * N + n) * P + p);
+    return e;
+}
+
+ST_HD inline void st_write_piece(const StQuad& c, int n, int b, int tile, const RowEnt* pix, int N, int P, int64_t Ppad,
+                                 RowEnt* rows, ExtRow* ext) {
+    const int p0 = c.x, Q0 = c.z, X0 = c.w & 0xFFFF, take = c.w >> 16;
+    const int x0 = X0 + n * (take + 2);
+    const RowEnt first = st_row(pix[p0], b, n, p0, N, P, Ppad);
+    ExtRow* e = ext + (size_t)tile * XR_EXT_ROWS + x0;
+    for (int k = 0; k < take + 2; ++k) e[k] = ExtRow{first.in_off + k, first.in_pitch};
+    RowEnt* r = rows + (size_t)tile * 256;
+    for (int k = 0; k < take; ++k) {
+        RowEnt q = st_row(pix[p0 + k], b, n, p0 + k, N, P, Ppad);
+        q.pad1 = x0 + k;
+        r[(Q0 + k) * N + n] = q;
+    }
+}
+
+ST_HD inline bool st_pad_row(const StQuad& ti, int r, int N) { return r >= ti.y * N; }
+ST_HD inline RowEnt st_invalid_row(const RowEnt& pix0) {
+    RowEnt e = pix0;
+    e.out_off = -1; e.pad0 = 0; e.pad1 = 0;
+    return e;
+}
+ST_HD inline ExtRow st_pad_ext(const StQuad& ti, int b, const RowEnt* pix, int N, int P, int64_t Ppad) {
+    const RowEnt first = st_row(pix[ti.x], b, 0, ti.x, N, P, Ppad);
+    return ExtRow{first.in_off, first.in_pitch};
+}
+
+inline int st_min_pixels(int N) {
+    const int Qmax = 256 / N;
+    return std::max(1, std::min(Qmax, (XR_EXT_ROWS - 3 * N) / (3 * N) + 1));
+}
diff --git a/bayes-od-rc_amd/engine.py b/bayes-od-rc_amd/engine.py
--- a/bayes-od-rc_amd/engine.py
+++ b/bayes-od-rc_amd/engine.py
@@ -378,11 +378,11 @@
         return out
 
     def plan_info(self):
-        info = (C.c_int32 * 8)()
-        self._chk(self.lib.bod_plan_info(self.h, info))
+        info = (C.c_int32 * 9)()
+        self._chk(self.lib.bod_plan_info_n(self.h, info, 9))
         return {"aggregating": bool(info[0]), "fused_head_outputs": bool(info[1]), "row_reuse": bool(info[2]),
                 "fan_out_row_reuse": bool(info[3]), "ops": int(info[4]), "plane_row_reuse_layers": int(info[5]), "tower_mx": bool(info[6]), "tower_mx_format": int(info[6]),
-                "sparse_tail": bool(info[7])}
+                "sparse_tail": bool(info[7]), "sparse_halo": bool(info[8])}
 
     @property
     def aggregating(self):
diff --git a/include/bayesod.h b/include/bayesod.h
--- a/include/bayesod.h
+++ b/include/bayesod.h
@@ -168,6 +168,7 @@
                                  float* gathered_host, float** gathered_device);
 
 bod_status bod_plan_info(bod_handle h, int32_t* info8);
+bod_status bod_plan_info_n(bod_handle h, int32_t* info, int32_t n);
 
 #ifdef __cplusplus
 }
diff --git a/include/bayesod_cdef.h b/include/bayesod_cdef.h
--- a/include/bayesod_cdef.h
+++ b/include/bayesod_cdef.h
@@ -134,3 +134,4 @@
 bod_status bod_gather_detections(bod_handle h, int32_t slot, void* nccl_comm, int32_t world, int32_t rank, int32_t root,
                                  float* gathered_host, float** gathered_device);
 bod_status bod_plan_info(bod_handle h, int32_t* info8);
+bod_status bod_plan_info_n(bod_handle h, int32_t* info, int32_t n);
```

After: 2217 images/sec, median of 6. +3.6%, better.
